# msalvaris/batchai_retinanet_horovod_coco

Measured on AMD Instinct MI355X. Metric: images/sec (whole node) RetinaNet-R50-FPN 800px at 1/2/4/8 MI355X, higher is better.
Workload: dtype bf16; 1 GPU; model=RetinaNet-R50-FPN, global_batch=16, per_gpu_batch=16, parallelism=dp1, clip_mode=global, allreduce_dtype=fp32, conv_backend=auto, hip_kernels=True, hip_graph=False, comm_engine=none, conv_table=/root/repo/tuning/conv_table.json, conv_raced=0, focal_fused_calls=101

## Files before the change

batchai_retinanet_horovod_coco_amd/models/retinanet.py:

```python
from __future__ import annotations

from typing import Dict, List, Optional, Sequence, Tuple

import os

import torch
import torch.nn as nn

from ..ops import anchors as anchor_ops
from ..ops import boxes as box_ops
from ..ops import conv as conv_ops
from ..ops import norm as norm_ops
from .layers import Conv2D, GroupNorm, prior_probability_bias
from .resnet import ResNet


class FPN(nn.Module):

    def __init__(self, c3: int, c4: int, c5: int, feature_size: int = 256):
        super().__init__()
        f = feature_size
        self.C5_reduced = Conv2D("C5_reduced", c5, f, 1, 1, "same")
        self.P5 = Conv2D("P5", f, f, 3, 1, "same")
        self.C4_reduced = Conv2D("C4_reduced", c4, f, 1, 1, "same")
        self.P4 = Conv2D("P4", f, f, 3, 1, "same")
        self.C3_reduced = Conv2D("C3_reduced", c3, f, 1, 1, "same")
        self.P3 = Conv2D("P3", f, f, 3, 1, "same")
        self.P6 = Conv2D("P6", c5, f, 3, 2, "same")
        self.P7 = Conv2D("P7", f, f, 3, 2, "same")

    def forward(self, C3, C4, C5, joins=None) -> List[torch.Tensor]:
        j = joins or {}
        P5r = self.C5_reduced(C5, join=j.get(3))
        P4m = conv_ops.upsample_add(P5r, self.C4_reduced(C4, join=j.get(2)))
        P3m = conv_ops.upsample_add(P4m, self.C3_reduced(C3, join=j.get(1)))
        P5 = self.P5(P5r)
        P4 = self.P4(P4m)
        P3 = self.P3(P3m)
        P6 = self.P6(C5, join=j.get(3))
        P7 = self.P7(torch.relu(P6))
        return [P3, P4, P5, P6, P7]

    def convs(self) -> List[Conv2D]:
        return [self.C5_reduced, self.P5, self.C4_reduced, self.P4, self.C3_reduced, self.P3, self.P6, self.P7]


HEAD_NORMS = (None, "gn")


def check_head_norm(head_norm, head_norm_groups: int, width: int = 256):
    if head_norm == "none":
        head_norm = None
    if head_norm not in HEAD_NORMS:
        raise ValueError("head_norm must be None or 'gn', got {!r}".format(head_norm))
    if head_norm == "gn" and (int(head_norm_groups) < 1 or width % int(head_norm_groups)):
        raise ValueError("head_norm_groups must divide the tower width {}, got {}".format(width, head_norm_groups))
    return head_norm


class Submodel(nn.Module):

    def __init__(self, name: str, prefix: str, cin: int, width: int, out_channels: int, final_bias: float,
                 head_norm: Optional[str] = None, head_norm_groups: int = 32):
        super().__init__()
        self.keras_name = name
        self.head_norm = check_head_norm(head_norm, head_norm_groups, width)
        self.tower = nn.ModuleList(
            [Conv2D(f"{prefix}_{i}", cin if i == 0 else width, width, 3, 1, "same", True, True, "normal001")
             for i in range(4)])
        self.final = Conv2D(prefix, width, out_channels, 3, 1, "same", True, False, "normal001", bias_value=final_bias)
        self.norms = None
        if self.head_norm == "gn":
            self.norms = nn.ModuleList([GroupNorm(f"{prefix}_{i}_gn", width, int(head_norm_groups)) for i in range(4)])
        if os.environ.get("MXR_HEAD_MAIN_WGRAD", "0") == "1":
            for c in self.convs():
                c.weight.mxr_main_wgrad = True

    def forward(self, feats: List[torch.Tensor]) -> List[torch.Tensor]:
        x = feats
        for i, c in enumerate(self.tower):
            w, b = c.effective(x[0].dtype)
            if self.norms is None:
                x = conv_ops.pyramid_conv(x, w, b, relu=True)
            else:
                n = self.norms[i]
                x = [norm_ops.group_norm_relu_nhwc(t, n.gamma, n.beta, n.groups, n.eps)
                     for t in conv_ops.pyramid_conv(x, w, b, relu=False)]
        w, b = self.final.effective(x[0].dtype)
        return conv_ops.pyramid_conv(x, w, b, relu=False)

    def forward_packed(self, x: torch.Tensor, shapes, pad_sink=None, join=None, chain=None) -> torch.Tensor:
        from ..ops import native_conv
        from ..ops import fp8
        if self.norms is not None:
            if fp8.enabled():
                raise RuntimeError("head_norm='gn' does not go with fp8: the tower layers hand fp8 copies of their "
                                   "ReLU outputs to each other")
            for i, (c, n) in enumerate(zip(self.tower, self.norms)):
                x = native_conv.pyramid_conv_layer(x, shapes, c, False, mask_input_grad=False, grad_premasked=False,
                                                   join=join if i == 0 else None, out_f8=False)
                x = norm_ops.group_norm_relu(x, shapes, n.gamma, n.beta, n.groups, n.eps)
            return native_conv.pyramid_conv_layer(x, shapes, self.final, False, mask_input_grad=False,
                                                  pad_sink=pad_sink)
        for i, c in enumerate(self.tower):
            nxt = self.tower[i + 1] if i + 1 < len(self.tower) else self.final
            x = native_conv.pyramid_conv_layer(x, shapes, c, True, mask_input_grad=i > 0, grad_premasked=True,
                                               join=join if i == 0 else None,
                                               out_f8=fp8.eligible(nxt.cin, nxt.cout),
                                               act=None if chain is None else (chain, len(self.tower) - i))
        return native_conv.pyramid_conv_layer(x, shapes, self.final, False, mask_input_grad=True,
                                              pad_sink=pad_sink, act=None if chain is None else (chain, 0))

    def convs(self) -> List[Conv2D]:
        return list(self.tower) + [self.final]


class RetinaNet(nn.Module):

    def __init__(self, num_classes: int, backbone: str = "resnet50", num_anchors: int = 9,
                 feature_size: int = 256, prior_probability: float = 0.01, head_norm: Optional[str] = None,
                 head_norm_groups: int = 32, regression_bins: int = 0, regression_range: float = 8.0):
        super().__init__()
        self.head_norm = check_head_norm(head_norm, head_norm_groups)
        self.head_norm_groups = int(head_norm_groups)
        self.regression_bins, self.regression_range = box_ops.check_regression_bins(regression_bins, regression_range)
        self.num_classes = num_classes
        self.num_anchors = num_anchors
        self.backbone_name = backbone
        if "resnet" in backbone:
            self.backbone = ResNet(backbone)
        else:
            from .extra_backbones import make_backbone
            self.backbone = make_backbone(backbone)
        c3, c4, c5 = self.backbone.out_channels[1:]
        self.fpn = FPN(c3, c4, c5, feature_size)
        self.regression_submodel = Submodel("regression_submodel", "pyramid_regression", feature_size, 256,
                                            num_anchors * 4 * max(1, self.regression_bins), 0.0, self.head_norm,
                                            self.head_norm_groups)
        self.classification_submodel = Submodel("classification_submodel", "pyramid_classification", feature_size,
                                                256, num_anchors * num_classes,
                                                prior_probability_bias(prior_probability), self.head_norm,
                                                self.head_norm_groups)

    def features(self, images: torch.Tensor) -> List[torch.Tensor]:
        joins = self._grad_joins(images)
        if joins is None:
            C3, C4, C5 = self.backbone(images)
            return self.fpn(C3, C4, C5)
        C3, C4, C5 = self.backbone(images, joins=joins)
        return self.fpn(C3, C4, C5, joins=joins if self.backbone.joins_active else None)

    def _grad_joins(self, images: torch.Tensor):
        if not (torch.is_grad_enabled() and isinstance(self.backbone, ResNet) and images.is_cuda
                and os.environ.get("MXR_GRAD_JOIN", "1") == "1" and conv_ops.get_conv_backend() != "torch"):
            return None
        from ..ops import native, native_conv
        if not native.available():
            return None
        dt = torch.bfloat16
        fpn = [self.fpn.C3_reduced, self.fpn.C4_reduced, self.fpn.C5_reduced, self.fpn.P6]
        if images.dtype != dt or not all(native_conv.hip_conv_ok(c.cin, c.cout, dt) for c in fpn):
            return None
        return {1: native_conv.GradJoin(2), 2: native_conv.GradJoin(2), 3: native_conv.GradJoin(2)}

    def forward(self, images: torch.Tensor) -> Dict[str, torch.Tensor]:
        feats = self.features(images)
        B = images.shape[0]
        if conv_ops.use_packed_heads(feats[0]):
            from ..ops import native
            packed, shapes = native.pyramid_pack(feats)
            from ..ops import native_conv
            join = native_conv.GradJoin(2) if (torch.is_grad_enabled() and
                                               os.environ.get("MXR_GRAD_JOIN", "1") == "1") else None
            self.reg_pad_sink = {} if torch.is_grad_enabled() else None
            from ..ops import fp8, row_activity
            chain = None
            if (torch.is_grad_enabled() and row_activity.enabled() and packed.dtype == torch.bfloat16
                    and self.head_norm is None and not fp8.enabled()):
                chain = row_activity.GradChain(len(self.regression_submodel.tower))
            reg = self.regression_submodel.forward_packed(packed, shapes, self.reg_pad_sink, join=join, chain=chain)
            self.cls_pad_sink = {} if torch.is_grad_enabled() else None
            req = getattr(self, "focal_request", None)
            if self.cls_pad_sink is not None and req is not None:
                self.cls_pad_sink["focal"] = req
            cls = self.classification_submodel.forward_packed(packed, shapes, self.cls_pad_sink, join=join)
            cls = cls.reshape(B, -1, self.num_classes)
            if self.regression_bins:
                return self._with_integral(reg.reshape(B, -1, 4 * self.regression_bins), cls)
            return {"regression": reg.reshape(B, -1, 4), "classification": cls}
        self.cls_pad_sink = self.reg_pad_sink = None
        reg = self.regression_submodel(feats)
        cls = self.classification_submodel(feats)
        classification = torch.cat([c.reshape(B, -1, self.num_classes) for c in cls], dim=1)
        if self.regression_bins:
            return self._with_integral(torch.cat([r.reshape(B, -1, 4 * self.regression_bins) for r in reg], dim=1),
                                       classification)
        regression = torch.cat([r.reshape(B, -1, 4) for r in reg], dim=1)
        return {"regression": regression, "classification": classification}

    def _with_integral(self, logits: torch.Tensor, classification: torch.Tensor) -> Dict[str, torch.Tensor]:
        K, R = self.regression_bins, self.regression_range
        state = getattr(self, "integral_request", None)
        if state is not None and logits.is_cuda:
            from ..ops import native
            try:
                regression = native.box_integral_fwd(logits.detach(), K, R, state=state)
                return {"regression": regression, "regression_logits": logits, "classification": classification}
            except native.NotServed:
                pass
        return {"regression": box_ops.box_integral(logits, K, R), "regression_logits": logits,
                "classification": classification}

    def convs(self) -> List[Conv2D]:
        return (self.backbone.convs() + self.fpn.convs() + self.regression_submodel.convs()
                + self.classification_submodel.convs())

    def pyramid_shapes(self, image_hw: Sequence[int]) -> List[Tuple[int, int]]:
        c = self.backbone.feature_shapes(image_hw)
        C3, C4, C5 = c[1], c[2], c[3]
        p6 = self.fpn.P6.out_hw(C5)
        p7 = self.fpn.P7.out_hw(p6)
        return [tuple(C3), tuple(C4), tuple(C5), tuple(p6), tuple(p7)]

    def backbone_parameters(self):
        return list(self.backbone.parameters())

    def norms(self) -> List[GroupNorm]:
        return [n for sub in (self.regression_submodel, self.classification_submodel) for n in (sub.norms or [])]

    def freeze_backbone(self) -> None:
        for p in self.backbone.parameters():
            p.requires_grad_(False)


class RetinaNetBBox(nn.Module):

    def __init__(self, model: RetinaNet, nms: bool = True, class_specific_filter: bool = True,
                 nms_threshold: float = 0.5, score_threshold: float = 0.05, max_detections: int = 300):
        super().__init__()
        self.model = model
        self.nms = nms
        self.class_specific_filter = class_specific_filter
        self.nms_threshold = nms_threshold
        self.score_threshold = score_threshold
        self.max_detections = max_detections
        self._anchors = anchor_ops.AnchorCache()

    @torch.no_grad()
    def forward(self, images: torch.Tensor):
        out = self.model(images)
        H, W = images.shape[1], images.shape[2]
        anchors = self._anchors.get((H, W), images.device, shapes_callback=anchor_ops.make_shapes_callback(self.model))
        from ..ops import native
        if (self.nms and self.class_specific_filter and images.is_cuda and native.available()
                and self.max_detections <= 512):
            return native.filter_detections_batched(anchors, out["regression"], out["classification"], H, W,
                                                    self.score_threshold, self.nms_threshold, self.max_detections)
        boxes = box_ops.bbox_transform_inv(anchors[None], out["regression"].float())
        boxes = box_ops.clip_boxes(boxes, H, W)
        cls = torch.sigmoid(out["classification"].float())
        res_b, res_s, res_l = [], [], []
        for i in range(images.shape[0]):
            b, s, l = box_ops.filter_detections(boxes[i], cls[i], self.nms, self.class_specific_filter,
                                                self.nms_threshold, self.score_threshold, self.max_detections)
            res_b.append(b)
            res_s.append(s)
            res_l.append(l)
        return torch.stack(res_b), torch.stack(res_s), torch.stack(res_l)


def retinanet_bbox(model: RetinaNet, **kwargs) -> RetinaNetBBox:
    return RetinaNetBBox(model, **kwargs)
```

batchai_retinanet_horovod_coco_amd/ops/conv_launch.py:

```python
from __future__ import annotations

import ctypes
import functools
import os
from typing import Callable, NamedTuple, Optional, Sequence, Tuple

import torch
import torch.nn.functional as F

from . import halo as _hx
from . import native as _n
from . import row_activity as _ra
from .native import ConvGeom, _chk, _p, _s, lib, zero_page, c_int, c_ll, c_vp
from .side_stream import SIDE


_SIGS = {
    "mxr_conv_wgrad": [c_vp, c_vp, c_int, c_vp, c_int, c_vp, c_vp, c_int, c_vp, ctypes.POINTER(ConvGeom), c_int, c_vp],
    "mxr_bias_grad": [c_vp, c_ll, c_int, c_int, c_int, c_vp, c_vp, c_vp, c_int, c_vp],
    "mxr_bias_res_act": [c_vp, c_vp, c_vp, c_ll, c_int, c_int, c_vp],
    "mxr_relu_bwd": [c_vp, c_vp, c_vp, c_ll, c_vp],
}

_BOUND = [False]
# ... 68 lines not shown
    @classmethod
    def of(cls, t: torch.Tensor) -> "BitMask":
        bm = cls(t)
        sh = torch.arange(8, device=t.device, dtype=torch.int32)
        bm.bits.copy_(((t.reshape(-1, 8) > 0).to(torch.int32) << sh).sum(1).to(torch.uint8))
        return bm

    def dense(self) -> torch.Tensor:
        sh = torch.arange(8, device=self.bits.device, dtype=torch.uint8)
        return ((self.bits[:, None] >> sh) & 1).bool().reshape(self.shape)

MASK_BITS = os.environ.get("MXR_MASK_BITS", "1") == "1"

FWD_VARIANTS = (0, 1, 2, 3, 4, 5, 6, 7, 8, 9, 10, 11, 12, 13, 14, 15, 16)
_IGEMM_VARIANTS = tuple(v for v in FWD_VARIANTS if v < 3)

def launch_hip(x, w, bias, res, y, g: ConvGeom, relu: bool, accumulate: bool = False, variant: int = 0,
               mask: Optional[torch.Tensor] = None) -> None:
    zp = _p(zero_page(x.device))
    if variant >= 3:
        return _chk(lib().mxr_conv_fwd_pipe(_p(x), _p(w), _p(bias), _p(res), _p(mask), _p(y), zp, ctypes.byref(g),
                                            int(relu), int(accumulate), variant - 3, _s()), "conv_fwd_pipe")
    _chk(lib().mxr_conv_fwd(_p(x), _p(w), _p(bias), _p(res), _p(mask), _p(y), zp, ctypes.byref(g), int(relu),
                            int(accumulate), variant, _s()), "conv_fwd")

HALO_VARIANTS = (0, 1, 2, 3, 4, 5, 6, 7, 8, 9, 10, 11, 12, 13, 14, 15)

HX32_VARIANTS = (0, 1, 2, 3, 4, 5, 6, 7, 8, 9, 10, 11, 12, 13, 14, 15)
HX32_NARROW = (8, 9)


NARROW_TILES = True


_HX32_WIDE = tuple(v for v in HX32_VARIANTS if v not in HX32_NARROW)

def hx32_variants(g: ConvGeom):
    return HX32_VARIANTS if g.cout <= 64 and NARROW_TILES else _HX32_WIDE

C1X1_BN = (64, 128, 256)

P8_VARIANTS = (0, 1, 2, 3, 4, 5, 6, 7, 8, 10)

P8_TUNED = (5, 6, 8)

def p8_covers(g: ConvGeom) -> bool:
    K = g.kh * g.kw * g.cin
    return (g.cin % 64 == 0 and g.cout % 8 == 0 and g.ostride == 1 and 1 <= g.nlev <= 5 and g.kh * g.kw <= 16
            and (int(g.M) + 1) * max(g.cin, g.cout) < 2 ** 31 and g.cout * K < 2 ** 31)

def big_tile_variants(g: ConvGeom):
    return ["p8_%d" % v for v in P8_TUNED] if p8_covers(g) else []

def launch_p8(x, w, bias, res, y, g: ConvGeom, relu: bool, accumulate: bool = False, variant: int = 0,
              mask: Optional[torch.Tensor] = None) -> None:
    if not p8_covers(g):
        raise RuntimeError("conv_p8: geometry not covered")
    K = g.kh * g.kw * g.cin
    if not (x.is_contiguous() and w.is_contiguous() and y.is_contiguous() and x.shape[-1] == g.cin
            and int(w.numel()) == g.cout * K and int(y.numel()) == int(g.M) * g.cout
            and (bias is None or bias.data_ptr() % 16 == 0)):
        raise RuntimeError("conv_p8: operand shapes do not match the geometry")
    _chk(lib().mxr_conv_p8(_p(x), _p(w), _p(bias), _p(res), _p(mask), _p(y), _p(zero_page(x.device)),
                           ctypes.byref(g), int(relu), int(accumulate), int(variant), _s()), "conv_p8")

SK_VARIANTS = (11, 12)


def splitk_splits(g: ConvGeom, v: int) -> int:
    if g.ostride != 1 or g.cin % 32 or g.cout % 8:
        return 0
    bco = 128 if v == 11 else 64
    tiles = -(-int(g.M) // 128) * -(-g.cout // bco)
    nks = g.kh * g.kw * g.cin // 32
    if tiles >= 256 or nks < 16:
        return 0
    s = min(64, max(2, round(512 / tiles)), nks // 8)
    return s if s >= 2 else 0


def launch_splitk(x, w, bias, res, y, g: ConvGeom, relu: bool, accumulate: bool = False, variant: int = 11,
                  mask: Optional[torch.Tensor] = None) -> None:
    ns = splitk_splits(g, variant)
    if ns < 2:
        raise RuntimeError("conv_fwd_pipe_sk: geometry not covered")
    part = torch.empty(ns * int(g.M) * g.cout, dtype=torch.float32, device=y.device)
    _chk(lib().mxr_conv_fwd_pipe_sk(_p(x), _p(w), _p(bias), _p(res), _p(mask), _p(y), _p(zero_page(x.device)),
                                    ctypes.byref(g), int(relu), int(accumulate), int(variant), ns, _p(part), _s()),
         "conv_fwd_pipe_sk")


def c1x1_variants(g: ConvGeom):
    if not (g.kh == 1 and g.kw == 1 and g.nlev == 1 and g.ostride == 1 and g.pt == 0 and g.pl == 0
            and g.stride in (1, 2) and g.cin in (64, 128, 256) and g.cout % 8 == 0):
        return []
    if g.stride == 1 and (g.H[0] != g.Ho[0] or g.W[0] != g.Wo[0]):
        return []
    eff = lambda bn: 64 if bn == 65 else bn
    return ["c1x1_%d" % bn for bn in C1X1_BN + (65,) if eff(bn) * g.cin <= 32768 and eff(bn) <= max(64, g.cout)]

def launch_c1x1(x, w, bias, res, y, g: ConvGeom, relu: bool, accumulate: bool = False, bn: int = 128,
                mask: Optional[torch.Tensor] = None) -> None:
    if "c1x1_%d" % bn not in c1x1_variants(g):
        raise RuntimeError("conv1x1_stream: geometry not covered")
    nimg = int(g.M) // (g.Ho[0] * g.Wo[0])
    if not (x.is_contiguous() and w.is_contiguous() and y.is_contiguous() and x.shape[-1] == g.cin
            and int(x.numel()) == nimg * g.H[0] * g.W[0] * g.cin and int(y.numel()) == int(g.M) * g.cout
            and int(w.numel()) == g.cout * g.cin and (bias is None or bias.data_ptr() % 16 == 0)):
        raise RuntimeError("conv1x1_stream: operand shapes do not match the geometry")
    _chk(lib().mxr_conv1x1_stream(_p(x), _p(w), _p(bias), _p(res), _p(mask), _p(y), int(g.M), g.cout, g.cin,
                                  g.H[0], g.W[0], g.Ho[0], g.Wo[0], g.stride, int(relu), int(accumulate), bn, 0,
                                  _s()), "conv1x1_stream")

def c1p_covers(g: ConvGeom) -> bool:
    return (g.kh == 1 and g.kw == 1 and g.nlev == 1 and g.ostride == 1 and g.pt == 0 and g.pl == 0
            and g.stride == 1 and g.H[0] == g.Ho[0] and g.W[0] == g.Wo[0] and g.cin % 32 == 0 and g.cin >= 96
            and g.cout % 8 == 0 and g.cout >= 64 and int(g.M) < 2 ** 31)

def launch_c1p(x, w, bias, res, y, g: ConvGeom, relu: bool, accumulate: bool = False,
               mask: Optional[torch.Tensor] = None) -> None:
    if not c1p_covers(g):
        raise RuntimeError("conv1x1_pers: geometry not covered")
    if not (x.is_contiguous() and w.is_contiguous() and y.is_contiguous() and x.shape[-1] == g.cin
            and int(x.numel()) == int(g.M) * g.cin and int(y.numel()) == int(g.M) * g.cout
            and int(w.numel()) == g.cout * g.cin and (bias is None or bias.data_ptr() % 16 == 0)
            and (res is None or (res.is_contiguous() and int(res.numel()) == int(g.M) * g.cout))):
        raise RuntimeError("conv1x1_pers: operand shapes do not match the geometry")
    _chk(lib().mxr_conv1x1_pers(_p(x), _p(w), _p(bias), _p(res), _p(mask), _p(y), _p(zero_page(x.device)),
                                _p(_n.trash_page(x.device)), int(g.M), g.cout, g.cin, int(relu), int(accumulate),
                                _s()), "conv1x1_pers")

def launch_halo(x, w, bias, res, y, g: ConvGeom, relu: bool, accumulate: bool = False, variant: int = 0,
                mask: Optional[torch.Tensor] = None) -> None:
    if not _hx.covers(g):
        raise RuntimeError("conv3x3_halo: geometry not covered")
    tiles, nt = _hx.device_tiles(_hx.geom_batch(g), _hx.geom_shapes(g), x.device)
    _chk(lib().mxr_conv3x3_halo(_p(x), _p(w), _p(bias), _p(res), _p(mask), _p(y), _p(zero_page(x.device)),
                                ctypes.byref(g), _p(tiles), nt, int(relu), int(accumulate), int(variant), _s()),
         "conv3x3_halo")

def launch_hx32(x, w, bias, res, y, g: ConvGeom, relu: bool, accumulate: bool = False, variant: int = 0,
                mask: Optional[torch.Tensor] = None, active=None) -> None:
    if not hx32_covers(g):
        raise RuntimeError("conv3x3_hx32: geometry not covered")
    if not (x.is_contiguous() and w.is_contiguous() and y.is_contiguous() and x.shape[-1] == g.cin
            and int(w.numel()) == g.cout * 9 * g.cin and int(y.numel()) == int(g.M) * g.cout
            and int(x.numel()) == int(g.M) * g.cin and (bias is None or bias.data_ptr() % 16 == 0)):
        raise RuntimeError("conv3x3_hx32: operand shapes do not match the geometry")
    if (g.cin // 32) % 2:
        variant = {2: 0, 3: 1, 13: 10, 14: 12}.get(variant, variant)
    tiles, nt = _hx.device_tiles(_hx.geom_batch(g), _hx.geom_shapes(g), x.device)
    wp = hx32_packed(w, g.cout, g.cin)
    act = active if active is not None else _ra.current()
    if act is not None and act.M == int(g.M) and act.ntiles == nt and bias is None and res is None and not relu:
        _ra.LAUNCHES["dgrad"] += 1
        return _chk(lib().mxr_conv3x3_hx32_act(_p(x), _p(wp), None, None, _p(mask), _p(y), _p(zero_page(x.device)),
                                               ctypes.byref(g), _p(tiles), nt, 0, int(accumulate), int(variant),
                                               _p(act.order), _p(act.count), _s()), "conv3x3_hx32_act")
    _chk(lib().mxr_conv3x3_hx32(_p(x), _p(wp), _p(bias), _p(res), _p(mask), _p(y), _p(zero_page(x.device)),
                                ctypes.byref(g), _p(tiles), nt, int(relu), int(accumulate), int(variant), _s()),
         "conv3x3_hx32")

class FocalRequest:

    def __init__(self, alpha: float = 0.25, gamma: float = 2.0):
        self.alpha, self.gamma = alpha, gamma
        self._buf = _n.ShapeSlots()
        self._qbuf = _n.ShapeSlots()
        self.set(None, None, None, 0)

    def set(self, state, label, npos, A: int) -> None:
        self.state, self.label, self.npos, self.A = state, label, npos, int(A)
        self.loss = None

    def dpad(self, n: int, p: int, ld: int, device) -> torch.Tensor:
        return self._buf.get((n, p, ld, str(device)),
                             lambda: torch.zeros((n, p, ld), dtype=torch.bfloat16, device=device))

    def dpad_q(self, n: int, p: int, ld: int, device) -> torch.Tensor:
        return self._qbuf.get((n, p, ld, str(device)),
                              lambda: torch.zeros((n, p, ld), dtype=torch.uint8, device=device))


FOCAL_FUSED = True
FOCAL_PREFER_MS = 0.15
FOCAL_LAUNCHES = [0]


FOCAL_VARIANTS = (0, 10)


def launch_hx32_focal(x, w, bias, g: ConvGeom, req: "FocalRequest", ld: int, variant: int = 0) -> torch.Tensor:
    from .losses import LOGIT_HI, LOGIT_LO
    N = int(g.M) // g.out_img
    C = g.cout // req.A
    if not (hx32_covers(g) and x.is_contiguous() and w.is_contiguous() and int(x.numel()) == int(g.M) * g.cin
            and int(w.numel()) == g.cout * 9 * g.cin and bias is not None and bias.data_ptr() % 16 == 0
            and C == 80 and req.gamma == 2.0 and ld % 8 == 0 and ld >= g.cout
            and int(req.state.numel()) == int(g.M) * req.A and int(req.label.numel()) == int(g.M) * req.A):
        raise RuntimeError("conv3x3_hx32_focal: operands do not match the geometry")
    tiles, nt = _hx.device_tiles(_hx.geom_batch(g), _hx.geom_shapes(g), x.device)
    wp = hx32_packed(w, g.cout, g.cin)
    nparts = -(-g.cout // 256) * nt
    parts = torch.empty(nparts, dtype=torch.float32, device=x.device)
    out = torch.empty(1, dtype=torch.float32, device=x.device)
    dpad = req.dpad(N, g.out_img, ld, x.device)
    if variant not in FOCAL_VARIANTS:
        raise RuntimeError("conv3x3_hx32_focal: no focal form of variant %r" % (variant,))
    _chk(lib().mxr_conv3x3_hx32_focal_v(_p(x), _p(wp), _p(bias), _p(zero_page(x.device)), ctypes.byref(g), _p(tiles),
                                        nt, _p(req.state.contiguous()), _p(req.label.contiguous()), _p(req.npos),
                                        _p(dpad), int(ld), req.A, C, float(req.alpha), float(req.gamma), LOGIT_LO,
                                        LOGIT_HI, _p(parts), nparts, _p(out), int(variant), _s()),
         "conv3x3_hx32_focal")
    req.loss = out.reshape(())
    FOCAL_LAUNCHES[0] += 1
    return dpad

def hx32_packed(w: torch.Tensor, cout: int, cin: int) -> torch.Tensor:
    cw = _n.compute_weights()
    if cw is not None:
        wp = cw.hx32_packed(w)
        if wp is not None:
            return wp
    wp = torch.empty(cout * 9 * cin, dtype=w.dtype, device=w.device)
    _chk(lib().mxr_hx32_pack_weights(_p(w), _p(wp), cout, cin, _s()), "hx32_pack")
    return wp

def hx32_covers(g: ConvGeom) -> bool:
    return _hx.covers(g) and g.cout * 9 * g.cin * 2 < 2 ** 31


class Family(NamedTuple):
    prefix: str
    names: Callable
    launch: Callable
    bits: object

def _numbered(prefix: str, fn):
    n = len(prefix)
    return lambda *a: fn(*a[:8], int(a[8][n:]), a[9])

@functools.lru_cache(maxsize=None)
def _named(prefix: str, variants) -> Tuple[str, ...]:
    return tuple("%s%d" % (prefix, v) for v in variants)

FAMILIES = (
    Family("hip", lambda g: _named("hip", FWD_VARIANTS if g.cout % 8 == 0 else _IGEMM_VARIANTS),
           _numbered("hip", launch_hip), lambda name: name[3:].isdigit() and int(name[3:]) >= 3),
    Family("halo", lambda g: _named("halo", HALO_VARIANTS) if _hx.covers(g) else (), _numbered("halo", launch_halo), True),
    Family("hx32_", lambda g: _named("hx32_", hx32_variants(g)) if hx32_covers(g) else (),
           _numbered("hx32_", launch_hx32), True),
    Family("c1x1_", c1x1_variants, _numbered("c1x1_", launch_c1x1), True),
    Family("c1p", lambda g: ("c1p",) if c1p_covers(g) else (), lambda *a: launch_c1p(*a[:8], a[9]), True),
    Family("p8_", big_tile_variants, _numbered("p8_", launch_p8), False),
    Family("sk", lambda g: _named("sk", tuple(v for v in SK_VARIANTS if splitk_splits(g, v))),
           _numbered("sk", launch_splitk), True),
)
_FAMILY = {f.prefix: f for f in FAMILIES}

FWD_ORDER = ("hip", "halo", "hx32_", "c1x1_", "c1p", "p8_", "sk")
DGRAD_ORDER = ("hip", "c1x1_", "c1p", "p8_", "halo", "hx32_")
DGRAD_S2_ORDER = ("hip",)
DGRAD_SKIP = ("c1x1_65",)

def family_of(name: str) -> Optional[Family]:
    return _FAMILY.get(name.rstrip("0123456789"))

def offered(g: ConvGeom, order=FWD_ORDER, skip=()):
    return [n for p in order for n in _FAMILY[p].names(g) if n not in skip]

def bits_capable(name: str) -> bool:
    bits = getattr(family_of(name), "bits", False)
    return bits(name) if callable(bits) else bits

def _bits_filter(cands, mask):
    if not isinstance(mask, BitMask):
        return cands
    return {k: v for k, v in cands.items() if bits_capable(k)}

def launch_fwd(x, w, bias, res, y, g: ConvGeom, relu: bool, accumulate: bool = False,
               variant=None, mask: Optional[torch.Tensor] = None) -> None:
    v = _variant(g.cout) if variant is None else variant
    if not isinstance(v, str):
        return launch_hip(x, w, bias, res, y, g, relu, accumulate, v, mask)
    fam = family_of(v)
    if fam is None:
        raise RuntimeError("launch_fwd: %r names no kernel family" % (v,))
    fam.launch(x, w, bias, res, y, g, relu, accumulate, v, mask)

def relu_bwd_(dy: torch.Tensor, y: torch.Tensor) -> torch.Tensor:
    assert dy.is_contiguous() and y.is_contiguous() and dy.shape == y.shape
    _chk(_bind().mxr_relu_bwd(_p(dy), _p(y), _p(dy), dy.numel(), _s()), "relu_bwd_")
    return dy

def relu_bwd(dy: torch.Tensor, y: torch.Tensor) -> torch.Tensor:
    dx = torch.empty_like(dy)
    _chk(_bind().mxr_relu_bwd(_p(dy), _p(y), _p(dx), dy.numel(), _s()), "relu_bwd")
    return dx

def bias_res_act_(y: torch.Tensor, bias: Optional[torch.Tensor], res: Optional[torch.Tensor], relu: bool):
    if bias is None and res is None and not relu:
        return y
    _chk(_bind().mxr_bias_res_act(_p(y), _p(bias), _p(res), y.numel(), y.shape[-1], int(relu), _s()), "epilogue")
    return y

def miopen_fwd(x, w, bias, res, stride, pads, relu):
    pt, pb, pl, pr = pads
# ... 206 lines not shown
```

batchai_retinanet_horovod_coco_amd/ops/halo.py:

```python
from __future__ import annotations

from typing import Dict, List, Sequence, Tuple

import numpy as np

HX_BOX = 4
HX_HMAX = 448
HX_PB = 256
COLMAX = 84
NFIELD = 10
TILE_INTS = 4 + HX_BOX * NFIELD


def _split(n: int, parts: int) -> List[Tuple[int, int]]:
    out, start = [], 0
    for i in range(parts):
        ln = n // parts + (1 if i < n % parts else 0)
        out.append((start, ln))
        start += ln
    return out


def level_boxes(H: int, W: int) -> List[Tuple[int, int, int, int]]:
    cols = _split(W, -(-W // COLMAX))
    cmax = max(c for _, c in cols)
    R = max(1, min(H, HX_PB // cmax))
    while R > 1 and (R + 2) * (cmax + 2) > HX_HMAX:
        R -= 1
    boxes = []
    for y0 in range(0, H, R):
        r = min(R, H - y0)
        for x0, c in cols:
            boxes.append((y0, r, x0, c))
    return boxes


def build_tiles(N: int, shapes: Sequence[Tuple[int, int]], open_tiles: int = 4) -> np.ndarray:
    img = sum(h * w for h, w in shapes)
    offs, o = [], 0
    for h, w in shapes:
        offs.append(o)
        o += h * w
    per_level = [level_boxes(h, w) for h, w in shapes]
    tiles: List[dict] = []
    open_idx: List[int] = []
    for b in range(N):
        for lv, (H, W) in enumerate(shapes):
            base = b * img + offs[lv]
            for (y0, R, x0, C) in per_level[lv]:
                ns, nh = R * C, (R + 2) * (C + 2)
                di = None
                for ti in open_idx:
                    t = tiles[ti]
                    if len(t["boxes"]) < HX_BOX and t["nslot"] + ns <= HX_PB and t["nhalo"] + nh <= HX_HMAX:
                        di = ti
                        break
                if di is None:
                    tiles.append({"boxes": [], "nslot": 0, "nhalo": 0})
                    di = len(tiles) - 1
                    open_idx.append(di)
                    if len(open_idx) > open_tiles:
                        open_idx.pop(0)
                t = tiles[di]
                t["boxes"].append((t["nslot"], t["nhalo"], base, base, H, W, y0, x0, R, C))
                t["nslot"] += ns
                t["nhalo"] += nh
                if (t["nslot"] > HX_PB - 16 or len(t["boxes"]) == HX_BOX) and di in open_idx:
                    open_idx.remove(di)
    out = np.zeros((len(tiles), TILE_INTS), dtype=np.int32)
    for i, t in enumerate(tiles):
        out[i, 0:3] = (len(t["boxes"]), t["nslot"], t["nhalo"])
        for k, bx in enumerate(t["boxes"]):
            out[i, 4 + k * NFIELD:4 + (k + 1) * NFIELD] = bx
    return out


def _boxes(row) -> List[Tuple[int, ...]]:
    return [tuple(int(v) for v in row[4 + k * NFIELD:4 + (k + 1) * NFIELD]) for k in range(int(row[0]))]


def check_tiles(tab: np.ndarray, N: int, shapes: Sequence[Tuple[int, int]]) -> None:
    total = N * sum(h * w for h, w in shapes)
    seen = np.zeros(total, dtype=np.int32)
    for row in tab:
        nbox, nslot, nhalo = int(row[0]), int(row[1]), int(row[2])
        assert 1 <= nbox <= HX_BOX and nslot <= HX_PB and nhalo <= HX_HMAX, row[:4]
        s = h = 0
        for (sbeg, hoff, ib, ob, H, W, y0, x0, R, C) in _boxes(row):
            assert sbeg == s and hoff == h and ib == ob
            assert 0 <= y0 and y0 + R <= H and 0 <= x0 and x0 + C <= W
            for r in range(R):
                seen[ob + (y0 + r) * W + x0:ob + (y0 + r) * W + x0 + C] += 1
            s += R * C
            h += (R + 2) * (C + 2)
        assert s == nslot and h == nhalo
    assert (seen == 1).all(), "pixels covered {} .. {} times".format(seen.min(), seen.max())


def waste(tab: np.ndarray, N: int, shapes: Sequence[Tuple[int, int]]) -> float:
    return 1.0 - N * sum(h * w for h, w in shapes) / float(len(tab) * HX_PB)


def emulate(x: np.ndarray, w: np.ndarray, tab: np.ndarray) -> np.ndarray:
    P, cin = x.shape
    cout = w.shape[0]
    y = np.zeros((P, cout), dtype=np.float64)
    for row in tab:
        nslot, nhalo = int(row[1]), int(row[2])
        boxes = _boxes(row)
        halo = np.zeros((HX_HMAX, cin))
        for h in range(nhalo):
            k = max(i for i in range(len(boxes)) if h >= boxes[i][1])
            sbeg, hoff, ib, ob, H, W, y0, x0, R, C = boxes[k]
            hr, hc = divmod(h - hoff, C + 2)
            yy, xx = y0 - 1 + hr, x0 - 1 + hc
            if 0 <= yy < H and 0 <= xx < W:
                halo[h] = x[ib + yy * W + xx]
        for p in range(nslot):
            k = max(i for i in range(len(boxes)) if p >= boxes[i][0])
            sbeg, hoff, ib, ob, H, W, y0, x0, R, C = boxes[k]
            r, c = divmod(p - sbeg, C)
            pw = C + 2
            hb = hoff + r * pw + c
            acc = np.zeros(cout)
            for ky in range(3):
                for kx in range(3):
                    acc += w[:, ky, kx, :] @ halo[hb + ky * pw + kx]
            y[ob + (y0 + r) * W + x0 + c] = acc
    return y



def pack_row_bits(rows: np.ndarray) -> np.ndarray:
    P = int(rows.shape[0])
    pad = np.zeros((P + 63) // 64 * 64, dtype=np.uint64)
    pad[:P] = rows.astype(np.uint64)
    return (pad.reshape(-1, 64) << np.arange(64, dtype=np.uint64)).sum(axis=1, dtype=np.uint64)


def unpack_row_bits(words: np.ndarray, P: int) -> np.ndarray:
    w = np.asarray(words).view(np.uint64).reshape(-1, 1)
    return ((w >> np.arange(64, dtype=np.uint64)) & np.uint64(1)).astype(bool).reshape(-1)[:P]


def dilate_rows(rows: np.ndarray, N: int, shapes: Sequence[Tuple[int, int]]) -> np.ndarray:
    out = np.zeros_like(rows, dtype=bool)
    img = sum(h * w for h, w in shapes)
    for b in range(N):
        off = b * img
        for h, w in shapes:
            a = rows[off:off + h * w].reshape(h, w).astype(bool)
            p = np.zeros((h + 2, w + 2), dtype=bool)
            p[1:-1, 1:-1] = a
            d = np.zeros((h, w), dtype=bool)
            for dy in range(3):
                for dx in range(3):
                    d |= p[dy:dy + h, dx:dx + w]
            out[off:off + h * w] = d.reshape(-1)
            off += h * w
    return out


def active_tiles(tab: np.ndarray, rows: np.ndarray) -> np.ndarray:
    act = np.zeros(len(tab), dtype=bool)
    for i, row in enumerate(tab):
        for (sbeg, hoff, ib, ob, H, W, y0, x0, R, C) in _boxes(row):
            ya, yb = max(0, y0 - 1), min(H - 1, y0 + R)
            xa, xb = max(0, x0 - 1), min(W - 1, x0 + C)
            lv = rows[ob:ob + H * W].reshape(H, W)
            if lv[ya:yb + 1, xa:xb + 1].any():
                act[i] = True
                break
    return act


def tile_rows(tab: np.ndarray, which: np.ndarray, P: int) -> np.ndarray:
    out = np.zeros(P, dtype=bool)
    for row in tab[np.asarray(which, dtype=bool)]:
        for (sbeg, hoff, ib, ob, H, W, y0, x0, R, C) in _boxes(row):
            for r in range(R):
                out[ob + (y0 + r) * W + x0:ob + (y0 + r) * W + x0 + C] = True
    return out


_CACHE: Dict[tuple, object] = {}


def device_tiles(N: int, shapes: Sequence[Tuple[int, int]], device):
    import torch
    key = (str(device), int(N), tuple((int(h), int(w)) for h, w in shapes), COLMAX)
    hit = _CACHE.get(key)
    if hit is None:
        tab = build_tiles(N, key[2])
        hit = (torch.from_numpy(tab).to(device), int(tab.shape[0]))
        _CACHE[key] = hit
    return hit


def geom_shapes(g) -> List[Tuple[int, int]]:
    return [(int(g.H[l]), int(g.W[l])) for l in range(int(g.nlev))]


def geom_batch(g) -> int:
    return int(g.M // max(1, g.out_img))


def covers(g) -> bool:
    if not (g.kh == 3 and g.kw == 3 and g.stride == 1 and g.pt == 1 and g.pl == 1 and g.ostride == 1):
        return False
    if g.cin % 32 or g.cout % 8:
        return False
    if any(g.H[l] != g.Ho[l] or g.W[l] != g.Wo[l] for l in range(g.nlev)):
        return False
    if g.in_img != g.out_img:
        return False
    return (g.M + 1) * max(g.cin, g.cout) < 2 ** 31
```

batchai_retinanet_horovod_coco_amd/ops/native.py:

```python
from __future__ import annotations

import ctypes
import os
from typing import List, Optional, Sequence, Tuple

import torch
import torch.nn.functional as F

_HERE = os.path.dirname(os.path.abspath(__file__))
_PKG = os.path.dirname(_HERE)
LIB_PATH = os.environ.get("MXR_KERNEL_LIB") or os.path.join(_PKG, "_lib", "libmxr_kernels.so")

_LIB: Optional[ctypes.CDLL] = None
_DISABLED = [os.environ.get("MXR_DISABLE_KERNELS", "0") == "1"]
_LOAD_ERR: List[str] = []

c_int, c_ll, c_float, c_vp = ctypes.c_int, ctypes.c_longlong, ctypes.c_float, ctypes.c_void_p

MAXLEV = 5


class ConvGeom(ctypes.Structure):
    _fields_ = [("nlev", c_int), ("H", c_int * MAXLEV), ("W", c_int * MAXLEV), ("Ho", c_int * MAXLEV),
                ("Wo", c_int * MAXLEV), ("in_off", c_int * MAXLEV), ("mstart", c_int * (MAXLEV + 1)),
                ("in_img", c_int), ("out_img", c_int), ("stride", c_int), ("pt", c_int), ("pl", c_int),
                ("kh", c_int), ("kw", c_int), ("cin", c_int), ("cout", c_int), ("M", c_ll),
                ("ostride", c_int), ("oH", c_int), ("oW", c_int), ("ooy", c_int), ("oox", c_int)]


_SIGS = {
    "mxr_focal_fwd_bwd": [c_vp, c_vp, c_vp, c_vp, c_vp, c_vp, c_vp, c_ll, c_int, c_float, c_float, c_float, c_float,
                          c_int, c_int, c_int, c_vp],
    "mxr_smooth_l1_fwd_bwd": [c_vp, c_vp, c_vp, c_vp, c_vp, c_vp, c_vp, c_ll, c_float, c_int, c_int, c_int, c_vp],
    "mxr_iou_loss_fwd_bwd": [c_vp, c_vp, c_vp, c_vp, c_vp, c_vp, c_vp, c_vp, c_ll, c_int, c_int, c_float, c_int, c_int,
                             c_int, c_vp],
    "mxr_quality_loss_fwd_bwd": [c_vp, c_vp, c_vp, c_vp, c_vp, c_vp, c_vp, c_vp, c_vp, c_vp, c_ll, c_int, c_int, c_int,
                                 c_int, c_int, c_int, c_vp],
    "mxr_box_integral_fwd": [c_vp, c_vp, c_vp, c_ll, c_int, c_float, c_int, c_vp],
    "mxr_box_dist_fwd_bwd": [c_vp, c_vp, c_vp, c_vp, c_vp, c_vp, c_vp, c_vp, c_ll, c_int, c_float, c_float, c_int, c_int,
                             c_int, c_vp],
    "mxr_loss_grid": [],
    "mxr_gn_chunk_rows": [],
    "mxr_gn_relu_fwd": [c_vp] * 7 + [c_ll, c_int, c_ll, c_int, c_int, c_float, c_int, ctypes.POINTER(c_int), c_int, c_vp],
    "mxr_gn_relu_bwd": [c_vp] * 10 + [c_ll, c_int, c_ll, c_int, c_int, c_int, ctypes.POINTER(c_int), c_int, c_vp],
    "mxr_anchor_targets": [c_vp, c_vp, c_int, c_vp, c_int, c_int, c_vp, c_vp, c_vp, c_vp, c_vp, c_vp, c_float, c_float,
                           c_float, c_vp],
    "mxr_atss_targets": [c_vp, c_vp, c_int, ctypes.POINTER(c_int), c_int, c_vp, c_int, c_int, c_vp, c_vp, c_int, c_vp,
                         c_vp, c_vp, c_vp, c_vp, c_vp, c_vp, c_float, c_vp],
    "mxr_chunk_struct_sizes": [c_vp],
    "mxr_adam_step": [c_vp, c_vp, c_vp, c_vp, c_vp, c_vp, c_vp, c_int, c_vp, c_vp, c_vp, c_vp, c_float, c_float,
                      c_float, c_vp],
    "mxr_sgd_step": [c_vp, c_vp, c_vp, c_vp, c_vp, c_vp, c_int, c_vp, c_vp, c_vp, c_vp, c_vp, c_int, c_vp],
    "mxr_refresh_copy": [c_vp, c_vp, c_vp, c_vp, c_int, c_vp, c_vp],
    "mxr_adam_step_ema": [c_vp, c_vp, c_vp, c_vp, c_vp, c_vp, c_vp, c_vp, c_int, c_vp, c_vp, c_vp, c_vp, c_float,
                          c_float, c_float, c_float, c_ll, c_vp],
    "mxr_sgd_step_ema": [c_vp, c_vp, c_vp, c_vp, c_vp, c_vp, c_vp, c_int, c_vp, c_vp, c_vp, c_vp, c_vp, c_int,
                         c_float, c_ll, c_vp],
    "mxr_swap_refresh": [c_vp, c_vp, c_vp, c_vp, c_vp, c_int, c_vp, c_vp],
    "mxr_grad_norm_clip": [c_vp, c_ll, c_vp, c_float, c_float, c_float, c_vp, c_vp],
    "mxr_scale_inplace": [c_vp, c_ll, c_vp, c_vp],
    "mxr_norm_grid": [],
    "mxr_maxpool_fwd": [c_vp, c_vp, c_vp] + [c_int] * 11 + [c_int, c_int, c_vp],
    "mxr_wgrad3x3_c64": [c_vp] * 5 + [c_int] * 4 + [c_vp],
    "mxr_wgrad_halo": [c_vp, c_vp, c_int, c_vp, c_int, c_int, c_int, c_int, c_vp, c_vp, c_vp, c_vp, c_vp, c_int, c_int, c_int,
                       c_vp, c_vp, c_vp, c_int, c_vp],
    "mxr_flip_batch": [c_vp, c_vp, c_vp, c_vp, c_int, c_vp],
    "mxr_conv1x1_stream": [c_vp] * 6 + [c_int] * 12 + [c_vp],
    "mxr_conv1x1_pers_dual": [c_vp] * 9 + [c_ll, c_int, c_int, c_int, c_int, c_int, c_int, c_int, c_int, c_vp],
    "mxr_conv1x1_pers": [c_vp] * 8 + [c_ll, c_int, c_int, c_int, c_int, c_vp],
    "mxr_conv_wgrad_p8_f8": [c_vp, c_vp, c_int, c_vp, c_vp, c_vp, c_int, c_vp, c_vp, c_int, c_vp,
                             ctypes.POINTER(ConvGeom), c_int, c_vp],
    "mxr_hx8_quant_pack_batch": [c_vp, c_int, c_int, c_vp],
    "mxr_conv_wgrad_p8_f8_bias": [c_vp, c_vp, c_int, c_vp, c_vp, c_vp, c_int, c_vp, c_vp, c_int, c_vp,
                                  ctypes.POINTER(ConvGeom), c_int, c_vp, c_int, c_vp],
    "mxr_stem_fwd": [c_vp, c_vp, c_vp, c_vp] + [c_int] * 8 + [c_vp],
    "mxr_stem_pool_fwd": [c_vp, c_vp, c_vp, c_vp, c_vp] + [c_int] * 11 + [c_vp],
    "mxr_stem_pack": [c_vp, c_vp, c_vp, c_vp],
    "mxr_stem_wgrad": [c_vp, c_vp, c_vp, c_vp, c_vp] + [c_int] * 8 + [c_vp] + [c_int] * 4 + [c_vp],
    "mxr_maxpool_bwd": [c_vp, c_vp, c_vp] + [c_int] * 10 + [c_int, c_vp],
    "mxr_upsample_add_fwd": [c_vp, c_vp, c_vp, c_vp, c_vp] + [c_int] * 6 + [c_int, c_vp],
    "mxr_upsample_bwd": [c_vp, c_vp, c_vp, c_vp] + [c_int] * 6 + [c_int, c_vp],
    "mxr_decode_clip": [c_vp, c_vp, c_int, c_vp, c_int, c_int, c_float, c_float, c_float, c_vp],
    "mxr_nms": [c_vp, c_int, c_float, c_int, c_vp, c_vp, c_vp, c_vp],
    "mxr_filter_select": [c_vp, c_int, c_int, c_int, c_int, c_float, c_vp, c_vp, c_int, c_vp],
    "mxr_filter_nms": [c_vp, c_vp, c_int, c_int, c_int, c_int, c_vp, c_vp, c_int, c_int, c_int, c_float, c_float,
                       c_float, c_float, c_int, c_vp, c_vp, c_vp, c_vp, c_vp],
    "mxr_conv_geom_size": [],
    "mxr_s2_stack_flip": [c_vp, c_vp, c_int, c_int, c_vp, c_vp],
    "mxr_conv_fwd": [c_vp, c_vp, c_vp, c_vp, c_vp, c_vp, c_vp, ctypes.POINTER(ConvGeom), c_int, c_int, c_int, c_vp],
    "mxr_conv_fwd_pipe": [c_vp, c_vp, c_vp, c_vp, c_vp, c_vp, c_vp, ctypes.POINTER(ConvGeom), c_int, c_int, c_int,
                          c_vp],
    "mxr_conv_fwd_pipe_dual": [c_vp, c_vp, c_int, c_int, c_int, c_int, c_int, c_vp, c_vp, c_vp, c_vp, c_vp, c_vp,
                               ctypes.POINTER(ConvGeom), c_int, c_int, c_vp],
    "mxr_conv_dgrad_pipe_dd": [c_vp, c_vp, c_vp, c_vp, c_vp, c_vp, c_int, c_int, c_int, c_int, c_int, c_int, c_vp,
                               ctypes.POINTER(ConvGeom), c_int, c_vp],
    "mxr_conv_fwd_pipe_sk": [c_vp, c_vp, c_vp, c_vp, c_vp, c_vp, c_vp, ctypes.POINTER(ConvGeom), c_int, c_int, c_int,
                             c_int, c_vp, c_vp],
    "mxr_conv_p8": [c_vp, c_vp, c_vp, c_vp, c_vp, c_vp, c_vp, ctypes.POINTER(ConvGeom), c_int, c_int, c_int, c_vp],
    "mxr_conv3x3_halo": [c_vp, c_vp, c_vp, c_vp, c_vp, c_vp, c_vp, ctypes.POINTER(ConvGeom), c_vp, c_int, c_int, c_int,
                         c_int, c_vp],
    "mxr_hx32_pack_weights": [c_vp, c_vp, c_int, c_int, c_vp],
    "mxr_hx32_pack_batch": [c_vp, c_int, c_vp, c_ll, c_vp],
    "mxr_conv3x3_hx32": [c_vp, c_vp, c_vp, c_vp, c_vp, c_vp, c_vp, ctypes.POINTER(ConvGeom), c_vp, c_int, c_int, c_int,
                         c_int, c_vp],
    "mxr_conv_wgrad_p8": [c_vp, c_vp, c_int, c_vp, c_int, c_vp, c_vp, c_int, c_vp, ctypes.POINTER(ConvGeom), c_int,
                          c_vp],
    "mxr_conv_wgrad_p8_dual": [c_vp, c_vp, c_int, c_vp, c_int, c_vp, c_int, c_vp, c_vp, c_vp, c_vp, c_int, c_vp,
                               ctypes.POINTER(ConvGeom), c_int, c_vp],
    "mxr_conv_wgrad_p8_bias": [c_vp, c_vp, c_int, c_vp, c_int, c_vp, c_vp, c_int, c_vp, ctypes.POINTER(ConvGeom),
                               c_int, c_vp, c_int, c_vp],
    "mxr_conv3x3_hx32_act": [c_vp, c_vp, c_vp, c_vp, c_vp, c_vp, c_vp, ctypes.POINTER(ConvGeom), c_vp, c_int, c_int,
                             c_int, c_int, c_vp, c_vp, c_vp],
    "mxr_conv_wgrad_p8_bias_act": [c_vp, c_vp, c_int, c_vp, c_int, c_vp, c_vp, c_int, c_vp, ctypes.POINTER(ConvGeom),
                                   c_int, c_vp, c_int, c_vp, c_vp],
    "mxr_rows_nonzero": [c_vp, c_ll, c_int, c_vp, c_vp],
    "mxr_rows_dilate": [c_vp, c_vp, c_int, c_ll, ctypes.POINTER(ConvGeom), c_vp],
    "mxr_halo_active_tiles": [c_vp, c_int, c_vp, c_ll, c_int, c_vp, c_vp, c_vp],
    "mxr_conv_wgrad_pipe": [c_vp, c_vp, c_int, c_vp, c_int, c_vp, c_vp, c_int, c_vp, ctypes.POINTER(ConvGeom), c_int,
                            c_vp],
    "mxr_conv_wgrad_pipe_direct": [c_vp, c_vp, c_int, c_vp, c_vp, c_int, c_vp, ctypes.POINTER(ConvGeom), c_int, c_vp],
    "mxr_flip_transpose": [c_vp, c_vp, c_int, c_int, c_int, c_int, c_vp],
    "mxr_image_warp_normalize": [c_vp, c_int, c_int, c_vp, c_int, c_int, c_vp, c_int, c_int, c_int, c_float, c_float,
                                 c_float, c_float, c_float, c_vp],
    "mxr_image_resize_into": [c_vp, c_int, c_int, c_vp, c_int, c_int, c_ll, c_int, c_vp],
    "mxr_image_batch_resize_normalize": [c_vp, c_ll, c_vp, c_int, c_vp, c_int, c_int, c_int, c_int, c_float, c_float,
                                         c_float, c_float, c_vp],
    "mxr_image_batch_warp_resize_normalize": [c_vp, c_ll, c_vp, c_vp, c_int, c_vp, c_int, c_int, c_int, c_int, c_int,
                                              c_int, c_float, c_float, c_float, c_float, c_float, c_vp],
    "mxr_detections_finish": [c_vp, c_vp, c_vp, c_vp, c_int, c_int, c_float, c_vp, c_vp, c_vp],
    "mxr_fp8_amax": [c_vp, c_ll, c_vp, c_vp],
    "mxr_fp8_quant": [c_vp, c_ll, c_vp, c_vp, c_vp, c_vp],
    "mxr_fp8_quant_rows": [c_vp, c_int, c_int, c_vp, c_vp, c_vp],
    "mxr_conv_fwd_f8": [c_vp, c_vp, c_vp, c_vp, c_vp, c_vp, c_vp, c_vp, ctypes.POINTER(ConvGeom), c_int, c_vp, c_vp,
                        c_vp, c_int, c_float, c_int, c_vp],
    "mxr_conv_p8_f8": [c_vp, c_vp, c_vp, c_vp, c_vp, c_vp, c_vp, c_vp, c_vp, ctypes.POINTER(ConvGeom), c_int, c_int,
                       c_vp, c_vp, c_vp, c_int, c_float, c_int, c_vp],
    "mxr_bf8_quant": [c_vp, c_ll, c_vp, c_vp, c_vp, c_vp],
    "mxr_quant_delayed": [c_vp, c_ll, c_vp, c_vp, c_int, c_float, c_vp, c_int, c_vp],
    "mxr_hx8_pack_weights": [c_vp, c_vp, c_int, c_int, c_vp],
    "mxr_hx8_quant_pack": [c_vp, c_int, c_int, c_vp, c_vp, c_vp],
    "mxr_conv3x3_hx32_f8": [c_vp, c_vp, c_vp, c_vp, c_vp, c_vp, c_vp, c_vp, c_vp, ctypes.POINTER(ConvGeom), c_vp, c_int,
                            c_int, c_int, c_vp, c_vp, c_vp, c_int, c_float, c_int, c_vp],
    "mxr_conv3x3_hx32_focal": [c_vp, c_vp, c_vp, c_vp, ctypes.POINTER(ConvGeom), c_vp, c_int, c_vp, c_vp, c_vp, c_vp,
                               c_int, c_int, c_int, c_float, c_float, c_float, c_float, c_vp, c_int, c_vp, c_vp],
    "mxr_conv3x3_hx32_focal_v": [c_vp, c_vp, c_vp, c_vp, ctypes.POINTER(ConvGeom), c_vp, c_int, c_vp, c_vp, c_vp, c_vp,
                                 c_int, c_int, c_int, c_float, c_float, c_float, c_float, c_vp, c_int, c_vp, c_int,
                                 c_vp],
    "mxr_conv3x3_hx32_f8_focal": [c_vp, c_vp, c_vp, c_vp, c_vp, c_vp, ctypes.POINTER(ConvGeom), c_vp, c_int, c_vp, c_vp,
                                  c_vp, c_vp, c_int, c_int, c_int, c_float, c_float, c_float, c_float, c_vp, c_int, c_vp,
                                  c_vp],
    "mxr_conv3x3_hx32_f8_focal_q": [c_vp, c_vp, c_vp, c_vp, c_vp, c_vp, ctypes.POINTER(ConvGeom), c_vp, c_int, c_vp,
                                    c_vp, c_vp, c_vp, c_int, c_int, c_int, c_float, c_float, c_float, c_float, c_vp,
                                    c_int, c_vp, c_vp, c_vp, c_vp, c_int, c_float, c_vp],
    "mxr_s2_shuffle": [c_vp, c_vp, c_vp, c_int, c_int, c_int, c_int, c_int, c_int, c_int, c_vp],
    "mxr_s2_stack": [c_vp, c_vp, c_int, c_int, c_vp, c_vp],
    "mxr_pyr_pack": [c_vp, c_vp, c_vp, c_int, c_int, c_int, c_int, c_vp],
    "mxr_pyr_pack_f8": [c_vp, c_vp, c_vp, c_int, c_int, c_int, c_vp, c_vp, c_vp, c_int, c_float, c_vp],
}
_OPTIONAL = {"mxr_conv_wgrad", "mxr_bias_grad", "mxr_relu_bwd"}


def load(required: bool = False, check_device: bool = True) -> bool:
    global _LIB
    if _LIB is not None:
        return True
    if not os.path.exists(LIB_PATH):
        msg = "HIP kernel library not built: {} (run python -m batchai_retinanet_horovod_coco_amd.build)".format(LIB_PATH)
        _LOAD_ERR.append(msg)
        if required:
            raise RuntimeError(msg)
        return False
    try:
        lib = ctypes.CDLL(LIB_PATH)
        for name, args in _SIGS.items():
            fn = getattr(lib, name)
            fn.argtypes = args
            fn.restype = c_int
        if lib.mxr_conv_geom_size() != ctypes.sizeof(ConvGeom):
            raise RuntimeError("ConvGeom layout mismatch ({} vs {})".format(lib.mxr_conv_geom_size(),
                                                                         ctypes.sizeof(ConvGeom)))
    except Exception as e:
        _LOAD_ERR.append(str(e))
        if required:
            raise
        return False
    _LIB = lib
    return True


def disable() -> None:
    _DISABLED[0] = True


def enable() -> None:
    _DISABLED[0] = False


def available() -> bool:
    if _DISABLED[0] or not torch.cuda.is_available():
        return False
    return load(required=os.environ.get("MXR_REQUIRE_KERNELS", "1") == "1")


def conv_supported() -> bool:
    return available() and os.environ.get("MXR_HIP_CONV", "1") == "1"


def loaded_libraries() -> List[str]:
    return [LIB_PATH] if _LIB is not None else []


def lib() -> ctypes.CDLL:
    if _LIB is None:
        load(required=True)
    return _LIB


_RAW_STREAM = getattr(torch._C, "_cuda_getCurrentRawStream", None)
_CUR_DEV = getattr(torch._C, "_cuda_getDevice", None)


def _s() -> int:
    if _RAW_STREAM is not None:
        return _RAW_STREAM(_CUR_DEV())
    return torch.cuda.current_stream().cuda_stream


def _p(t: Optional[torch.Tensor]):
    return None if t is None else t.data_ptr()


_SYNC_DEBUG = os.environ.get("MXR_SYNC_DEBUG", "0") == "1"


def _chk(rc: int, name: str) -> None:
    if rc != 0:
        raise RuntimeError("{} failed with code {}".format(name, rc))
    if _SYNC_DEBUG:
        try:
            torch.cuda.synchronize()
        except RuntimeError as e:
            raise RuntimeError("{} faulted: {}".format(name, e)) from e


def _dt(t: torch.Tensor) -> int:
    if t.dtype == torch.bfloat16:
        return 1
    if t.dtype == torch.float32:
        return 0
    raise TypeError("unsupported dtype {}".format(t.dtype))


_ZERO = {}


def zero_page(device) -> torch.Tensor:
    key = str(device)
    z = _ZERO.get(key)
    if z is None:
        z = torch.zeros(256, dtype=torch.uint8, device=device)
        _ZERO[key] = z
    return z


_TRASH = {}


def trash_page(device) -> torch.Tensor:
    key = str(device)
    t = _TRASH.get(key)
# ... 1119 lines not shown
```

batchai_retinanet_horovod_coco_amd/ops/native_conv.py:

```python
from __future__ import annotations

import ctypes
import os
from typing import Optional, Sequence, Tuple

import torch
import torch.nn.functional as F

from . import native as _n
from .native import ConvGeom, _chk, _p, _s, lib, zero_page, c_int, c_ll, c_vp
from .side_stream import SIDE
from . import row_activity as _ra
from .conv_launch import (
    MASK_BITS, BitMask, bits_capable, proj_fusable, run_fwd_proj, run_fwd_into, C1X1_BN, FWD_VARIANTS, HALO_VARIANTS, HX32_VARIANTS, P8_TUNED, P8_VARIANTS, _BOUND, _SIGS, _bind,
    _effective, _miopen_pyramid_wgrad, _miopen_wgrad, _only, _out_hw, _variant, bias_res_act_,
    big_tile_variants, c1x1_variants, family_of, flip, fwd_candidates, geom_pyramid, geom_single, hip_conv_ok,
    hx32_covers, hx32_packed, launch_c1x1, launch_fwd, launch_halo, launch_hx32, launch_p8, miopen_fwd,
    p8_covers, relu_bwd, relu_bwd_, run_fwd, torch_conv_backward,)
from .conv_dgrad import (
    proj_dgrad_fusable, run_dgrad_proj, _dgrad_cands, _dgrad_s2_subpixel, _pick_taps, _s2_phase_taps, _s2_stack_taps,
    _s2_stacked_weights, _s2_stacked_weights_hip, conv_dgrad, run_dgrad,)
from .conv_wgrad import (
    proj_wgrad_fusable, run_wgrad_proj, _WGRAD_P8, _WGRAD_PIPE_OCC, _WGRAD_PIPE_TILE, _WGRAD_TILE, _WGRAD_VS, _WH_TILES, _deliver_wgrad,
    _only_wgrad, _sink, _splits, _splits_pipe, _wgrad_sink_cands, _wh_box, bias_grad, conv_wgrad,
# ... 134 lines not shown
                    h = run_fwd_proj(h, x, w2c, w1, b2c + b1, st1, emit=emit)
                else:
                    shortcut = run_fwd(x, w1, b1, None, st1, specs[nconv][1], False)
                    h = run_fwd(h, w2c, b2c, shortcut, st, pd, True, emit=emit)
            else:
                h = run_fwd(h, ws[i][0], ws[i][1], shortcut if last else None, st, pd, True, emit=emit if last else None)
            hs.append(h)
        if emit is not None:
            h._mxr_bits = emit
        ctx.specs = specs
        ctx.nconv = nconv
        ctx.has_b1 = specs[nconv] is not None
        ctx.wparams = [params[3 * i] for i in range(nconv + 1)]
        present = [i for i in range(nconv + 1) if ws[i] is not None]
        ctx.save_for_backward(*(hs + [ws[i][0] for i in present] + [scales[i] for i in present]))
        return h

    @staticmethod
    def backward(ctx, dout):
        specs, nconv = ctx.specs, ctx.nconv
        saved = ctx.saved_tensors
        hs = saved[:nconv + 1]
        nw = nconv + (1 if ctx.has_b1 else 0)
        ws = list(saved[nconv + 1:nconv + 1 + nw])
        scs = list(saved[nconv + 1 + nw:])
        out = hs[-1]
        g = dout.to(out.dtype).contiguous()
        if not ctx.premasked:
            g = relu_bwd(g, out)
        elif g is dout and not ctx.has_b1 and ctx.needs_input_grad[0] and not _INPLACE_GRAD:
            g = g.clone()
        grads = [None] * (3 * (nconv + 1))
        need_x = ctx.needs_input_grad[0]
        dx = None
        jbuf, mask_in = None, ctx.mask_in
        if ctx.join is not None and need_x:
            jbuf, _ = ctx.join.claim()
            mask_in = True
        dh_last = None
        wfused = False
        if ctx.has_b1:
            st, pd = specs[nconv]
            if (ctx.needs_input_grad[4 + 3 * nconv] and ctx.needs_input_grad[4 + 3 * (nconv - 1)] and nconv >= 2
                    and specs[nconv - 1] == (1, (0, 0, 0, 0)) and pd == (0, 0, 0, 0)
                    and proj_wgrad_fusable(hs[nconv - 1], hs[0], g, ws[nconv - 1], ws[nconv], st)):
                wfused = run_wgrad_proj(hs[nconv - 1], hs[0], g, st, scs[nconv - 1], scs[nconv],
                                        ctx.wparams[nconv - 1], ctx.wparams[nconv])
            if ctx.needs_input_grad[4 + 3 * nconv] and not wfused:
                grads[3 * nconv] = run_wgrad(hs[0], g, ws[nconv], st, pd, scs[nconv], param=ctx.wparams[nconv])
            if need_x:
                if (nconv >= 2 and specs[nconv - 1] == (1, (0, 0, 0, 0)) and pd == (0, 0, 0, 0) and
                        proj_dgrad_fusable(g, ws[nconv - 1], ws[nconv], hs[nconv - 1], tuple(hs[0].shape), st)):
                    dh_last, dx = run_dgrad_proj(g, ws[nconv - 1], ws[nconv], hs[nconv - 1], tuple(hs[0].shape), st,
                                                 out=jbuf)
                else:
                    dx = run_dgrad(g, ws[nconv], hs[0], st, pd, out=jbuf)
        gi = g
        for i in range(nconv - 1, -1, -1):
            st, pd = specs[i]
            if ctx.needs_input_grad[4 + 3 * i] and not (wfused and i == nconv - 1):
                grads[3 * i] = run_wgrad(hs[i], gi, ws[i], st, pd, scs[i], param=ctx.wparams[i])
            if i > 0:
                if i == nconv - 1 and dh_last is not None:
                    gi = dh_last
                    continue
                gi = run_dgrad(gi, ws[i], hs[i], st, pd, mask=hs[i])
            elif need_x:
                mk = hs[0] if mask_in else None
                if mk is not None and ctx.bits_in is not None and ws[0].shape[1] == 1:
                    mk = ctx.bits_in
                if dx is None and jbuf is None and st == 1 and SIDE.usable(g):
                    dx = run_dgrad(gi, ws[0], hs[0], st, pd, res=g, mask=mk)
                else:
                    if dx is None:
                        if jbuf is not None:
                            dx = jbuf.add_(g)
                        else:
                            dx = g if gi is not g else g.clone()
                    dx = run_dgrad(gi, ws[0], hs[0], st, pd, out=dx, mask=mk)
        if ctx.join is not None and need_x:
            if jbuf is None:
                ctx.join.buf = dx
            else:
                if dx is not jbuf:
                    jbuf.copy_(dx)
                ctx.join.release()
                dx = None
        return (dx, None, None, None) + tuple(grads)

_BLOCK_CHUNK = int(os.environ.get("MXR_BLOCK_CHUNK", "0"))
_BLOCK_CHUNK_MIN_PX = int(os.environ.get("MXR_BLOCK_CHUNK_MIN_PX", "10000"))


def _block_chunk(x, specs) -> int:
    if (_BLOCK_CHUNK <= 0 or specs[-1] is not None or x.shape[0] < 2 * _BLOCK_CHUNK
            or x.shape[1] * x.shape[2] < _BLOCK_CHUNK_MIN_PX or any(st != 1 for st, _ in specs[:-1])):
        return 0
    return _BLOCK_CHUNK


def _bits_view(full: BitMask, i0: int, i1: int) -> BitMask:
    v = BitMask.__new__(BitMask)
    per = full.bits.numel() // full.shape[0]
    v.bits = full.bits[i0 * per:i1 * per]
    v.shape = (i1 - i0,) + tuple(full.shape[1:])
    v.device = full.device
    return v


def _chunked_chain(x, ws, specs, nconv, cout, bits_ok, chunk):
    N, H, W, _ = x.shape
    outs = [torch.empty((N, H, W, ws[i][0].shape[0]), dtype=x.dtype, device=x.device) for i in range(nconv)]
    emit = BitMask(shape=(N, H, W, cout), device=x.device) if bits_ok else None
    for i0 in range(0, N, chunk):
        i1 = min(N, i0 + chunk)
        xs = x[i0:i1]
        h = xs
        for i in range(nconv):
            st, pd = specs[i]
            last = i == nconv - 1
            em = _bits_view(emit, i0, i1) if (last and emit is not None) else None
            h = run_fwd_into(outs[i][i0:i1], h, ws[i][0], ws[i][1], xs if last else None, st, pd, True, emit=em)
    if emit is not None:
        outs[-1]._mxr_bits = emit
    return outs


def residual_block(x, convs, branch1, mask_input_grad: bool = False, grad_premasked: bool = False,
                   join: Optional[GradJoin] = None) -> torch.Tensor:
    specs, params = [], []
    hw = tuple(x.shape[1:3])
    for c in convs:
        specs.append((c.stride, tuple(c.pads(hw))))
        hw = c.out_hw(hw)
    specs.append(None if branch1 is None else (branch1.stride, tuple(branch1.pads(tuple(x.shape[1:3])))))
    for c in list(convs) + [branch1]:
        if c is None:
            params += [None, None, None]
            continue
        sc, sh = c.bn.scale_shift() if c.bn is not None else (None, None)
        params += [c.weight, sc, sh]
    return ResidualBlockFn.apply(x, tuple(specs), (bool(mask_input_grad), bool(grad_premasked)), join, *params)

def fused_block_ok(x, convs) -> bool:
    return (os.environ.get("MXR_FUSED_BLOCKS", "1") == "1" and x.is_cuda and x.dtype == torch.bfloat16
            and all(c is None or (hip_conv_ok(c.cin, c.cout, x.dtype) and c.bias is None) for c in convs))

HEAD_BITS = True

class PyramidConvFn(torch.autograd.Function):

    @staticmethod
    def forward(ctx, x, weight, bias, shapes, relu, mask_input_grad=False, grad_premasked=False, pad_sink=None,
                join=None, out_f8=False, act=None):
        from .conv_tuner import TUNER
        ctx.act = act
        x = x.contiguous()
        N, P, cin = x.shape
        cout = weight.shape[0]
        w, b = _effective(weight, None, bias, None)
        ctx.wdt = weight.dtype
        g = geom_pyramid(N, shapes, cin, cout)
        from . import fp8 as _f8
        ctx.f8x = None
        f8_only_in = getattr(x, "_mxr_f8only", False)
        ctx.bits_in = getattr(x, "_mxr_bits", None) if mask_input_grad else None
        if f8_only_in and not (_f8.enabled() and _f8.eligible(cin, cout) and _f8.WGRAD and ctx.bits_in is not None):
            raise RuntimeError("PyramidConvFn: the input is an fp8-only tower output; this layer would read its bf16 "
                               "values")
        if _f8.enabled() and _f8.eligible(cin, cout):
            from . import conv_launch as _cl
            req = pad_sink.get("focal") if pad_sink is not None else None
            if not (req is not None and req.state is not None and _cl.FOCAL_FUSED and req.A > 0):
                req = None
            y = _f8.pyramid_forward(x, w, b, g, relu, (N, P, cout), weight,
                                    TUNER.key("pfwd", N, tuple(shapes), cin, cout, int(relu)) + "|f8",
                                    f8_only=bool(out_f8) and _f8.WGRAD and _f8.F8_ONLY_TOWERS and MASK_BITS
                                    and relu and any(ctx.needs_input_grad), focal=req,
                                    focal_dq_ok=bool(weight.requires_grad and _f8.WGRAD
                                                     and (bias is None or _f8.bias_fusable(weight, bias))))
            if getattr(y, "_mxr_focal_dpad", None) is not None:
                pad_sink["dy"] = y._mxr_focal_dpad
            if weight.requires_grad and _f8.WGRAD:
                ctx.f8x = _f8.quantize_cached(x)
                if getattr(y, "_mxr_f8only", False):
                    y._mxr_grad_f8ok = bias is None or _f8.bias_fusable(weight, bias)
        elif _focal_fused(pad_sink, relu, b, g, TUNER.key("pfwd", N, tuple(shapes), cin, cout, int(relu))):
            from .conv_launch import launch_hx32_focal
            req = pad_sink["focal"]
            fv = 10 if TUNER.winner(TUNER.key("pfwd", N, tuple(shapes), cin, cout, int(relu))) == "hx32_10" else 0
            pad_sink["dy"] = launch_hx32_focal(x, w, b, g, req, (cout + 63) // 64 * 64, variant=fv)
            y = torch.empty((N, P, cout), dtype=x.dtype, device=x.device)
            y._mxr_unwritten = True
        else:
            emit = BitMask(shape=(N, P, cout), device=x.device) if (
                relu and MASK_BITS and HEAD_BITS and x.is_cuda and cout % 8 == 0 and any(ctx.needs_input_grad)) else None
            key = TUNER.key("pfwd", N, tuple(shapes), cin, cout, int(relu)) + ("|eb" if emit is not None else "")
            cands = fwd_candidates(x, w, b, None, g, 1, (1, 1, 1, 1), relu, (N, P, cout), allow_miopen=False,
                                   mask=emit)
            if cout % 8 and cout < 64:
                cands["pad64"] = lambda: _pad64_pfwd(x, w, b, shapes, relu)
            y = TUNER.run(key, cands)
            if emit is not None:
                y._mxr_bits = emit
        ctx.save_for_backward(x, w, y if relu else None)
        ctx.params = (weight, bias)
        ctx.cfg = (tuple(shapes), relu, bias is not None, bool(mask_input_grad), bool(grad_premasked))
        ctx.pad_sink = pad_sink
        ctx.join = join
        return y

    @staticmethod
    def backward(ctx, dy):
        from .conv_tuner import TUNER
        x, w, y = ctx.saved_tensors
        shapes, relu, has_bias, mask_in, premasked = ctx.cfg
        N, P, cin = x.shape
        cout = w.shape[0]
        padded = ctx.pad_sink.pop("dy", None) if ctx.pad_sink is not None else None
        if padded is not None:
            dy = padded
        else:
            dy = dy.to(x.dtype).contiguous()
        from . import fp8 as _f8
        dy_f8only = getattr(dy, "_mxr_f8only", False)
        if dy_f8only and not ((premasked or not relu) and ctx.f8x is not None and _f8.cache_get(dy) is not None
                              and (not has_bias or _f8.bias_fusable(ctx.params[0], ctx.params[1]))):
            raise RuntimeError("PyramidConvFn: the incoming gradient is an fp8-only data gradient; this layer would "
                               "read its bf16 values")
        if relu and not premasked:
            dy = relu_bwd(dy, y)
        dx = dw = db = None
        mk = None
        if mask_in:
            mk = ctx.bits_in if ctx.bits_in is not None else x
        ract = wact = None
        if ctx.act is not None and ctx.f8x is None:
            chain, depth_k = ctx.act
            if depth_k == 0:
                chain.start(dy, N, shapes)
            ract = chain.level(depth_k)
            wact = ract if depth_k > 0 else None
        f8_only_in = getattr(x, "_mxr_f8only", False)
        from . import fp8 as _f8
        f8dy = None
        if ctx.f8x is not None and ctx.needs_input_grad[1]:
            dq_src = dy
            if cout % 64 and dq_src.shape[-1] % 64:
                cp = (cout + 63) // 64 * 64
                dq_src = F.pad(dy, (0, cp - dy.shape[-1]))
            f8dy = _f8.quantize_bf8_cached(dq_src, key=("dyq", ctx.params[0]))
            if ctx.needs_input_grad[0] and cout % 64 and dq_src is not dy:
                dy = dq_src
        if ctx.needs_input_grad[0]:
            wd = flip(w)
            dyp = dy
            if cout % 64:
                cp = (cout + 63) // 64 * 64
                if dyp.shape[-1] != cp:
                    dyp = F.pad(dy, (0, cp - cout))
                wd = F.pad(wd, (0, cp - cout))
            wd = wd.contiguous()
            gd = geom_pyramid(N, shapes, dyp.shape[-1], cin)
            key = TUNER.key("pdgrad", N, tuple(shapes), cin, cout) + ("|mb" if isinstance(mk, BitMask) else "")
            buf = None
            if ctx.join is not None:
                buf, _ = ctx.join.claim()
            from . import fp8 as _f8
            if _f8.enabled() and _f8.dgrad_eligible(dyp.shape[-1], cin):
                f8o = f8_only_in and _f8.F8_ONLY_DGRAD and getattr(x, "_mxr_grad_f8ok", False)
                r = _f8.pyramid_dgrad(dyp, wd, gd, mk, (N, P, cin), ("pdgrad", ctx.params[0]),
                                      key + ("|a" if buf is not None else "") + "|f8", emit=mask_in, out=buf,
                                      f8_only=f8o)
                if buf is None:
                    dx = r
                    if ctx.join is not None:
                        ctx.join.buf = dx
                else:
                    ctx.join.release()
                    dx = None
            elif buf is None:
                with _ra.using(ract):
                    dx = TUNER.run(key, fwd_candidates(dyp, wd, None, None, gd, 1, (1, 1, 1, 1), False, (N, P, cin),
                                                       allow_miopen=False, mask=mk))
                if ctx.join is not None:
                    ctx.join.buf = dx
            else:
                cands = fwd_candidates(dyp, wd, None, None, gd, 1, (1, 1, 1, 1), False, (N, P, cin),
                                       allow_miopen=False, mask=mk, out=buf)
                if TUNER.needs_tuning(key + "|a", cands):
                    TUNER.run(key + "|a", fwd_candidates(dyp, wd, None, None, gd, 1, (1, 1, 1, 1), False,
                                                         (N, P, cin), allow_miopen=False, mask=mk, out=buf.clone()))
                with _ra.using(ract):
                    TUNER.run(key + "|a", cands)
                ctx.join.release()
                dx = None
        fused_bias = False
        if ctx.needs_input_grad[1]:
            gw = geom_pyramid(N, shapes, cin, cout)
            wkey = TUNER.key("pwgrad", N, tuple(shapes), cin, cout)
            if f8dy is not None and _f8.wgrad_eligible(gw, int(f8dy[0].shape[-1])):
                fb = has_bias and ctx.needs_input_grad[2] and _f8.bias_fusable(ctx.params[0], ctx.params[1])
                dw = _f8.deliver_pyramid_wgrad(ctx.f8x, f8dy, gw, ctx.params[0], reads=(x, dy),
                                               bias_param=ctx.params[1] if fb else None)
                if dw is not None:
                    dw = dw.to(ctx.wdt)
                if has_bias and ctx.needs_input_grad[2] and not fb:
                    db = deliver_bias_grad(ctx.params[1], dy, channels=cout)
                return dx, dw, db, None, None, None, None, None, None, None, None
            with _ra.using(wact):
                fused_bias = (has_bias and ctx.needs_input_grad[2]
                              and deliver_wgrad_bias_fused(wkey, x, dy, gw, ctx.params[0], ctx.params[1]))
        if f8_only_in and ctx.needs_input_grad[1]:
            raise RuntimeError("PyramidConvFn: a bf16 weight gradient over an fp8-only tower output")
        if ctx.needs_input_grad[1] and not fused_bias:
            cands = wgrad_candidates(x, dy, gw, None)
            dyl = dy if dy.shape[-1] == cout else dy[..., :cout]
            lib_fn = lambda: _miopen_pyramid_wgrad(x, w, dyl, shapes)
            cands["miopen"] = lib_fn
            sink_make = _wgrad_sink_cands(x, dy, gw, None, lib_fn)
            if cout % 8 and cout < 64:
                narrow = {"pad64": lambda: _pad64_pwgrad(x, dy, shapes, cout)}
                if SWAP_NARROW_WGRAD:
                    narrow["swap"] = lambda: _swap_pwgrad(x, dy, shapes, cout)
                cands.update(narrow)
                base_make = sink_make

                def sink_make(sink, only=None, base_make=base_make, narrow=narrow):
                    if only in narrow:
                        return {only: lambda: sink.add_(narrow[only]())}
                    c = base_make(sink, only)
                    if only is None:
                        c.update({n: (lambda fn=fn: sink.add_(fn())) for n, fn in narrow.items()})
                    return c
            with _ra.using(wact):
                dw = _deliver_wgrad(wkey, cands, sink_make, ctx.params[0], (x, dy))
            if dw is not None:
                dw = dw.to(ctx.wdt)
        if has_bias and ctx.needs_input_grad[2] and not fused_bias:
            db = deliver_bias_grad(ctx.params[1], dy, channels=cout)
        return dx, dw, db, None, None, None, None, None, None, None, None

def _focal_fused(pad_sink, relu, b, g: ConvGeom, key: str) -> bool:
    from . import conv_launch as _cl
    from .conv_tuner import TUNER
    req = pad_sink.get("focal") if pad_sink is not None else None
    return (req is not None and req.state is not None and _cl.FOCAL_FUSED and not relu and b is not None
            and req.A > 0 and g.cout == 80 * req.A and _cl.hx32_covers(g)
            and (TUNER.prefer(key, "hx32_10", _cl.FOCAL_PREFER_MS) or TUNER.prefer(key, "hx32_0", _cl.FOCAL_PREFER_MS)))

def _pad64_pfwd(x, w, b, shapes, relu):
    from .conv_tuner import TUNER
    N, P, cin = x.shape
    cout = w.shape[0]
    wp = F.pad(w, (0, 0, 0, 0, 0, 0, 0, 64 - cout)).contiguous()
    bp = None if b is None else F.pad(b, (0, 64 - cout)).contiguous()
    gp = geom_pyramid(N, shapes, cin, 64)
    yp = TUNER.run(TUNER.key("pfwd", N, tuple(shapes), cin, 64, int(relu), "pad"),
                   fwd_candidates(x, wp, bp, None, gp, 1, (1, 1, 1, 1), relu, (N, P, 64), allow_miopen=False))
    return yp[..., :cout].contiguous()

def _pad64_pwgrad(x, dy, shapes, cout):
    from .conv_tuner import TUNER
    N, P, cin = x.shape
    dyp = dy if dy.shape[-1] == 64 else F.pad(dy[..., :cout], (0, 64 - cout)).contiguous()
    gp = geom_pyramid(N, shapes, cin, 64)
    dw = TUNER.run(TUNER.key("pwgrad", N, tuple(shapes), cin, 64, "pad"), wgrad_candidates(x, dyp, gp, None))
    return dw[:cout]

SWAP_NARROW_WGRAD = True

def _swap_pwgrad(x, dy, shapes, cout):
    from .conv_tuner import TUNER
    N, P, cin = x.shape
    dyp = dy if dy.shape[-1] == 64 else F.pad(dy[..., :cout], (0, 64 - cout)).contiguous()
    gs = geom_pyramid(N, shapes, 64, cin)
    r = TUNER.run(TUNER.key("pwgrad", N, tuple(shapes), 64, cin, "swap"), wgrad_candidates(dyp, x, gs, None))
    return r[..., :cout].flip(1, 2).permute(3, 1, 2, 0)

def conv_layer(x, layer, residual=None, relu=None, join: Optional[GradJoin] = None) -> torch.Tensor:
    relu = layer.relu if relu is None else relu
    pads = layer.pads(x.shape[1:3])
    scale = shift = None
    if layer.bn is not None:
        scale, shift = layer.bn.scale_shift()
    if not hip_conv_ok(layer.cin, layer.cout, x.dtype):
        if join is not None:
            raise RuntimeError("GradJoin consumer %s is not on the HIP conv path" % layer.keras_name)
        from .conv import _conv_torch
        w, b = layer.effective(x.dtype)
        return _conv_torch(x, w, b, layer.stride, pads, relu, residual)
    return ConvLayerFn.apply(x, layer.weight, layer.bias, scale, shift, layer.stride, tuple(pads), bool(relu),
                             residual, join)

def _pyr_pack(packed: torch.Tensor, levels, shapes, unpack: bool) -> None:
    ptrs = (c_vp * 5)(*([t.data_ptr() for t in levels] + [None] * (5 - len(levels))))
    hw = (c_int * 5)(*([h * w for h, w in shapes] + [0] * (5 - len(shapes))))
    _chk(lib().mxr_pyr_pack(_p(packed), ptrs, hw, len(levels), packed.shape[0], packed.shape[-1], int(unpack), _s()),
         "pyr_pack")

class PyramidPackFn(torch.autograd.Function):

    @staticmethod
    def forward(ctx, *xs):
        N, C = xs[0].shape[0], xs[0].shape[-1]
        shapes = tuple((int(x.shape[1]), int(x.shape[2])) for x in xs)
        ctx.shapes = shapes
        packed = torch.empty((N, sum(h * w for h, w in shapes), C), dtype=xs[0].dtype, device=xs[0].device)
        from . import fp8 as _f8
        if _f8.enabled():
            st = _f8.amax_state("pyr_features", packed.device)
            yq = torch.empty(packed.shape, dtype=torch.uint8, device=packed.device) if st.ready else None
            inv = torch.empty(1, dtype=torch.float32, device=packed.device)
            levels = [x.contiguous() for x in xs]
            ptrs = (c_vp * 5)(*([t.data_ptr() for t in levels] + [None] * (5 - len(levels))))
            hw = (c_int * 5)(*([h * w for h, w in shapes] + [0] * (5 - len(shapes))))
            _chk(lib().mxr_pyr_pack_f8(_p(packed), ptrs, hw, len(levels), N, C, _p(yq), _p(st.amax3), _p(inv),
                                       int(st.phase), float(_f8.MARGIN), _s()), "pyr_pack_f8")
            if yq is not None:
                _f8.cache_put(packed, yq, inv)
            st.advance()
            return packed
        _pyr_pack(packed, [x.contiguous() for x in xs], shapes, False)
        return packed

    @staticmethod
    def backward(ctx, dp):
        dp = dp.contiguous()
        N, C = dp.shape[0], dp.shape[-1]
        outs = [torch.empty((N, h, w, C), dtype=dp.dtype, device=dp.device) for h, w in ctx.shapes]
        _pyr_pack(dp, outs, ctx.shapes, True)
        return tuple(outs)

def pyramid_pack(xs: Sequence[torch.Tensor]):
    N = xs[0].shape[0]
    C = xs[0].shape[-1]
    shapes = tuple((int(x.shape[1]), int(x.shape[2])) for x in xs)
    if (xs[0].is_cuda and xs[0].dtype == torch.bfloat16 and C % 8 == 0 and 1 <= len(xs) <= 5
            and all(x.dtype == xs[0].dtype and x.shape[0] == N and x.shape[-1] == C for x in xs)):
        return PyramidPackFn.apply(*xs), shapes
    packed = torch.cat([x.reshape(N, -1, C) for x in xs], dim=1)
    return packed, shapes

def pyramid_conv_layer(x, shapes, layer, relu, mask_input_grad=False, grad_premasked=False,
                       pad_sink=None, join=None, out_f8: bool = False, act=None) -> torch.Tensor:
    return PyramidConvFn.apply(x, layer.weight, layer.bias, tuple(shapes), bool(relu), bool(mask_input_grad),
                               bool(grad_premasked), pad_sink, join, bool(out_f8), act)

def pyramid_unpack(y, shapes):
    out, off = [], 0
    N = y.shape[0]
    for (h, wd) in shapes:
        out.append(y[:, off:off + h * wd].reshape(N, h, wd, -1))
        off += h * wd
    return out



class _RawConvFn(torch.autograd.Function):
    @staticmethod
    def forward(ctx, x, w, bias, stride, pads, relu, residual):
        ctx.wdt = w.dtype
        return ConvLayerFn.forward(ctx, x, w.float(), bias, None, None, stride, pads, relu, residual)

    @staticmethod
    def backward(ctx, dy):
        dx, dw, db, *_rest, dres = ConvLayerFn.backward(ctx, dy)
        return dx, (None if dw is None else dw.to(ctx.wdt)), db, None, None, None, dres

def conv2d(x, w, bias, stride, pads, relu, residual):
    if not hip_conv_ok(x.shape[-1], w.shape[0], x.dtype):
        from .conv import _conv_torch
        return _conv_torch(x, w, bias, stride, pads, relu, residual)
    return _RawConvFn.apply(x, w, bias, stride, tuple(pads), bool(relu), residual)

def pyramid_conv_packed(x, shapes, w, bias, relu):
    return PyramidConvFn.apply(x, w, bias, tuple(shapes), bool(relu))

def pyramid_conv(xs, w, bias, relu):
    packed, shapes = pyramid_pack(xs)
    return pyramid_unpack(pyramid_conv_packed(packed, shapes, w, bias, relu), shapes)
```

batchai_retinanet_horovod_coco_amd/ops/row_activity.py:

```python
from __future__ import annotations

import ctypes
import os
from typing import Dict, Optional, Sequence, Tuple

import torch

from . import halo as _hx
from .native import ConvGeom, _chk, _p, _s, lib

MAX_DEPTH = 8
LAUNCHES = {"dgrad": 0, "wgrad": 0}


def enabled() -> bool:
    return os.environ.get("MXR_SPARSE_REG_GRAD", "1") == "1"


class Activity:
    __slots__ = ("words", "order", "count", "M", "ntiles")

    def __init__(self, words, order, count, M, ntiles):
        self.words, self.order, self.count, self.M, self.ntiles = words, order, count, int(M), int(ntiles)


_CUR = [None]


class using:
    __slots__ = ("act", "prev")

    def __init__(self, act: Optional[Activity]):
        self.act, self.prev = act, None

    def __enter__(self):
        self.prev, _CUR[0] = _CUR[0], self.act
        return self.act

    def __exit__(self, *exc):
        _CUR[0] = self.prev
        return False


def current() -> Optional[Activity]:
    return _CUR[0]


def rows_nonzero(dy: torch.Tensor, out: Optional[torch.Tensor] = None) -> torch.Tensor:
    ld = int(dy.shape[-1])
    rows = dy.numel() // ld
    if not (dy.is_cuda and dy.dtype == torch.bfloat16 and dy.is_contiguous() and ld % 8 == 0):
        raise RuntimeError("rows_nonzero: a contiguous bf16 tensor with ld % 8 == 0")
    if out is None:
        out = torch.empty((rows + 63) // 64, dtype=torch.int64, device=dy.device)
    _chk(lib().mxr_rows_nonzero(_p(dy), rows, ld, _p(out), _s()), "rows_nonzero")
    return out


def rows_dilate(words: torch.Tensor, g: ConvGeom, nd: int = 1, out: Optional[torch.Tensor] = None) -> torch.Tensor:
    nw = (int(g.M) + 63) // 64
    if out is None:
        out = torch.empty((nd, nw), dtype=torch.int64, device=words.device)
    if not (words.numel() >= nw and out.is_contiguous() and tuple(out.shape) == (nd, nw)):
        raise RuntimeError("rows_dilate: mask sizes do not match the geometry")
    _chk(lib().mxr_rows_dilate(_p(words), _p(out), nd, nw, ctypes.byref(g), _s()), "rows_dilate")
    return out


def halo_active_tiles(tiles: torch.Tensor, ntiles: int, masks: torch.Tensor,
                      out: Optional[Tuple[torch.Tensor, torch.Tensor]] = None):
    k = int(masks.shape[0])
    if out is None:
        out = (torch.empty((k, ntiles), dtype=torch.int32, device=masks.device),
               torch.empty(k, dtype=torch.int32, device=masks.device))
    _chk(lib().mxr_halo_active_tiles(_p(tiles), ntiles, _p(masks), int(masks.shape[1]), k, _p(out[0]), _p(out[1]),
                                     _s()), "halo_active_tiles")
    return out


_WS: Dict[tuple, tuple] = {}


def _workspace(device, N: int, shapes, depth: int, nw: int, ntiles: int):
    key = (str(device), int(N), tuple(shapes), int(depth))
    ws = _WS.get(key)
    if ws is None:
        ws = (torch.zeros((depth + 1, nw), dtype=torch.int64, device=device),
              torch.zeros((depth + 1, ntiles), dtype=torch.int32, device=device),
              torch.zeros(depth + 1, dtype=torch.int32, device=device))
        _WS[key] = ws
    return ws


class GradChain:

    def __init__(self, depth: int):
        self.depth = int(depth)
        self.acts = None

    def start(self, dy: torch.Tensor, N: int, shapes: Sequence[Tuple[int, int]]) -> None:
        from .conv_launch import geom_pyramid
        self.acts = None
        ld = int(dy.shape[-1])
        if not (dy.is_cuda and dy.dtype == torch.bfloat16 and dy.is_contiguous() and ld % 8 == 0
                and 0 <= self.depth <= MAX_DEPTH):
            return
        shapes = tuple((int(h), int(w)) for h, w in shapes)
        g = geom_pyramid(N, shapes, 32, 32)
        if dy.numel() != int(g.M) * ld:
            return
        nw = (int(g.M) + 63) // 64
        tiles, nt = _hx.device_tiles(N, shapes, dy.device)
        masks, order, count = _workspace(dy.device, N, shapes, self.depth, nw, nt)
        rows_nonzero(dy, out=masks[0])
        if self.depth:
            rows_dilate(masks[0], g, self.depth, out=masks[1:])
        halo_active_tiles(tiles, nt, masks, out=(order, count))
        self.acts = [Activity(masks[k], order[k], count[k:k + 1], g.M, nt) for k in range(self.depth + 1)]

    def level(self, k: int) -> Optional[Activity]:
        if self.acts is None or not 0 <= k <= self.depth:
            return None
        return self.acts[k]
```

batchai_retinanet_horovod_coco_amd/train/engine.py:

```python
from __future__ import annotations

import contextlib
import os
from typing import Dict, Optional

import torch

from ..ops import anchors as anchor_ops
from ..ops import losses
from ..parallel import runtime
from ..parallel.distributed_optimizer import DistributedOptimizer
from .flat import FlatParams, backward_order
from .optimizer import KerasAdam, KerasSGD


_ROCTX = os.environ.get("MXR_ROCTX", "0") == "1"


class _range:

    def __init__(self, name: str):
        self.name = name

    def __enter__(self):
        if _ROCTX and torch.cuda.is_available():
            torch.cuda.nvtx.range_push(self.name)
        return self

    def __exit__(self, *a):
        if _ROCTX and torch.cuda.is_available():
            torch.cuda.nvtx.range_pop()


_PAD_FOCAL = os.environ.get("MXR_PAD_FOCAL", "1") == "1"

class Trainer:
    def __init__(self, model, lr: float = 1e-5, clipnorm: float = 0.001, compute_dtype: torch.dtype = torch.float32,
                 clip_mode: str = "local", compression=None, bucket_bytes: Optional[int] = None,
                 device: Optional[torch.device] = None, overlap: bool = True, target_backend: str = "auto",
                 optimizer: str = "adam", momentum: float = 0.0, nesterov: bool = False, weight_decay: float = 0.0,
                 ema_decay: float = 0.0, regression_loss: str = "smooth_l1", regression_weight: float = 1.0,
                 assigner: str = "iou", atss_topk: int = anchor_ops.ATSS_TOPK, classification_loss: str = "focal",
                 dfl_weight: float = losses.DFL_WEIGHT):
        from ..parallel.collectives import Compression
        self.regression_bins = int(getattr(model, "regression_bins", 0) or 0)
        self.regression_range = float(getattr(model, "regression_range", 8.0))
        if not self.regression_bins and dfl_weight != losses.DFL_WEIGHT:
            raise ValueError("dfl_weight goes with a distribution box head (regression_bins); this model has none")
        if not float(dfl_weight) >= 0:
            raise ValueError("dfl_weight must be >= 0, got {}".format(dfl_weight))
        self.dfl_weight = float(dfl_weight)
        if self.regression_bins:
            from ..ops import fp8 as _fp8
            if _fp8.enabled():
                raise ValueError("regression_bins={} does not go with fp8: the regression final's {} outputs would run "
                                 "in fp8".format(self.regression_bins, 4 * self.regression_bins * model.num_anchors))
        if classification_loss != "focal" and classification_loss not in losses.CLS_KINDS:
            raise ValueError("classification_loss must be 'focal' or one of {}, got {!r}".format(
                losses.CLS_KINDS, classification_loss))
        if classification_loss != "focal":
            from ..ops import fp8 as _fp8
            if _fp8.enabled():
                raise ValueError("classification_loss={!r} does not go with fp8: the classification final's focal loss "
                                 "is part of the fp8 epilogue".format(classification_loss))
        self.classification_loss = classification_loss
        if getattr(model, "head_norm", None) is not None:
            from ..ops import fp8 as _fp8
            if _fp8.enabled():
                raise ValueError("head_norm={!r} does not go with fp8: the fp8 tower layers hand fp8 copies of their "
                                 "ReLU outputs to each other".format(model.head_norm))
        if assigner not in ("iou", "atss"):
            raise ValueError("assigner must be 'iou' or 'atss', got {!r}".format(assigner))
        if assigner == "iou" and atss_topk != anchor_ops.ATSS_TOPK:
            raise ValueError("atss_topk goes with assigner='atss'; the fixed-threshold rule has no top-k")
        self.assigner = assigner
        self.atss_topk = anchor_ops._check_topk(atss_topk)
        if regression_loss != "smooth_l1" and regression_loss not in losses.IOU_KINDS:
            raise ValueError("regression_loss must be 'smooth_l1' or one of {}, got {!r}".format(
                losses.IOU_KINDS, regression_loss))
        if regression_loss == "smooth_l1" and regression_weight != 1.0:
            raise ValueError("regression_weight goes with the IoU regression losses; smooth_l1 has no weight")
        self.regression_loss = regression_loss
        self.regression_weight = float(regression_weight)
        self.device = device or (runtime.device() if runtime.is_initialized() else torch.device("cpu"))
        self.model = model.to(self.device)
        self.compute_dtype = compute_dtype
        self.flat = FlatParams(backward_order(self.model), device=self.device)
        if optimizer == "adam":
            if momentum or nesterov or weight_decay:
                raise ValueError("momentum, nesterov and weight_decay belong to optimizer='sgd'")
            self.base_optimizer = KerasAdam(self.flat, lr=lr, clipnorm=clipnorm, ema_decay=ema_decay)
        elif optimizer == "sgd":
            self.base_optimizer = KerasSGD(self.flat, lr=lr, momentum=momentum, nesterov=nesterov,
                                           weight_decay=weight_decay, clipnorm=clipnorm, ema_decay=ema_decay)
        else:
            raise ValueError("optimizer must be 'adam' or 'sgd', got {!r}".format(optimizer))
        self.optimizer = DistributedOptimizer(self.base_optimizer, compression=compression or Compression.none,
                                              clip_mode=clip_mode, bucket_bytes=bucket_bytes, overlap=overlap)
        if regression_loss != "smooth_l1":
            self.base_optimizer.regression_loss = regression_loss
            self.base_optimizer.regression_weight = self.regression_weight
        if classification_loss != "focal":
            self.base_optimizer.classification_loss = classification_loss
        if assigner != "iou":
            self.base_optimizer.assigner = assigner
            self.base_optimizer.atss_topk = self.atss_topk
        if self.dfl_weight != losses.DFL_WEIGHT:
            self.base_optimizer.dfl_weight = self.dfl_weight
        self.anchors = anchor_ops.AnchorCache()
        self.num_classes = model.num_classes
        self.target_backend = target_backend
        self.stop_training = False
        self.shapes_callback = None
        self.last_logs: Dict[str, torch.Tensor] = {}
        self.compute_weights = None
        self._ema_swapped = False
        from ..ops import native
        self._cls_pad_buf = native.ShapeSlots()
        self._focal_req = None
        self._reg_pad_buf = native.ShapeSlots()
        self.step_graphs = None
        from ..ops import fp8 as _fp8
        _fp8.reset_state()
        if (self.device.type == "cuda" and compute_dtype == torch.bfloat16 and native.available()
                and hasattr(self.model, "convs") and os.environ.get("MXR_NO_COMPUTE_WEIGHTS") != "1"):
            self.compute_weights = native.ComputeWeights(self.flat, self.model.convs())
            native.set_compute_weights(self.compute_weights)
        if self.device.type == "cuda" and native.available() and os.environ.get("MXR_NO_GRAD_SINKS") != "1":
            native.set_grad_sinks(native.GradSinks(self.flat, self.optimizer.notify_grad_ready))

    def compute_targets(self, images: torch.Tensor, gt: torch.Tensor, gt_count: torch.Tensor, image_hw: torch.Tensor):
        H, W = int(images.shape[1]), int(images.shape[2])
        anchors = self.anchors.get((H, W), self.device, self.shapes_callback)
        centers = self.anchors.centers((H, W), self.device, self.shapes_callback)
        from ..ops import native
        use_hip = (self.target_backend == "hip" or
                   (self.target_backend == "auto" and anchors.is_cuda and native.available()))
        if self.assigner == "atss":
            levels = self.anchors.levels((H, W), self.device, self.shapes_callback)
            if use_hip:
                return native.atss_targets(anchors, levels, gt, gt_count, image_hw, topk=self.atss_topk, centers=centers)
            state, label, reg = anchor_ops.atss_targets_torch(anchors, levels, gt, gt_count, image_hw,
                                                              topk=self.atss_topk, centers=centers)
            return state, label, reg, (state == 1).sum().to(torch.int32).reshape(1)
        if use_hip:
            return native.anchor_targets(anchors, gt, gt_count, image_hw, centers=centers)
        state, label, reg = anchor_ops.anchor_targets_torch(anchors, gt, gt_count, image_hw, centers=centers)
        return state, label, reg, (state == 1).sum().to(torch.int32).reshape(1)

    def _fused_losses(self) -> bool:
        from ..ops import native
        return self.device.type == "cuda" and native.available()

    def forward_backward(self, images, gt, gt_count, image_hw):
        with _range("targets"):
            state, label, reg_t, npos = self.compute_targets(images, gt, gt_count, image_hw)
        x = images.to(self.compute_dtype)
        req = self._focal_request(state, label, npos)
        if self.regression_bins and self._fused_losses():
            self.model.integral_request = state
        with _range("forward"):
            try:
                out = self.model(x)
            finally:
                if req is not None:
                    self.model.focal_request = None
                if self.regression_bins:
                    self.model.integral_request = None
        with _range("backward"):
            return self._losses_backward(out, reg_t, state, label, npos, self._loss_anchors(images))

    def _loss_anchors(self, images):
        if self.regression_loss == "smooth_l1" and self.classification_loss == "focal":
            return None
        return self.anchors.get((int(images.shape[1]), int(images.shape[2])), self.device, self.shapes_callback)

    def _regression_fwd_bwd(self, reg, reg_t, state, npos, anchors, **pad):
        from ..ops import native
        if self.regression_loss == "smooth_l1":
            return native.smooth_l1_fwd_bwd(reg, reg_t, state, npos, **pad)
        return native.iou_loss_fwd_bwd(reg, reg_t, anchors, state, npos, kind=self.regression_loss,
                                       weight=self.regression_weight, **pad)

    def _regression_torch(self, reg, reg_t, state, anchors):
        if self.regression_loss == "smooth_l1":
            return losses.smooth_l1_loss(reg, reg_t, state, backend="torch")
        return losses.iou_loss(reg, reg_t, state, anchors, self.regression_loss, self.regression_weight,
                               backend="torch")

    def _regression_terms_torch(self, out, reg_t, state, anchors):
        loss = self._regression_torch(out["regression"], reg_t, state, anchors)
        if self.regression_bins:
            loss = loss + losses.distribution_focal_loss(out["regression_logits"], reg_t, state, self.regression_bins,
                                                         self.regression_range, self.dfl_weight, backend="torch")
        return loss

    def _dist_losses_fused(self, out, reg_t, state, npos, anchors, A, rsink):
        from ..ops import native
        from ..ops import fp8 as _fp8
        if _fp8.enabled():
            raise RuntimeError("regression_bins={} does not go with fp8".format(self.regression_bins))
        K, R = self.regression_bins, self.regression_range
        logits, reg = out["regression_logits"], out["regression"]
        if reg.requires_grad:
            loss = self._regression_terms_torch(out, reg_t, state, anchors)
            return loss, loss, None
        box_loss, dreg = self._regression_fwd_bwd(reg, reg_t, state, npos, anchors)
        W = 4 * K * A
        if rsink is not None and _PAD_FOCAL and logits.dtype == torch.bfloat16 and logits.shape[1] % A == 0 and W % 64:
            key = (logits.shape[0], logits.shape[1] // A, (W + 63) // 64 * 64, logits.device)
            buf = self._reg_pad_buf.get(key, lambda: torch.zeros(key[:3], dtype=logits.dtype, device=logits.device))
            dfl, dpad = native.box_dist_fwd_bwd(logits.detach(), dreg, reg_t, state, npos, K, R, self.dfl_weight,
                                                grad_out=buf, group=A)
            rsink["dy"] = dpad
            dlog = torch.zeros((), dtype=logits.dtype, device=logits.device).expand(logits.shape)
        else:
            dfl, dlog = native.box_dist_fwd_bwd(logits.detach(), dreg, reg_t, state, npos, K, R, self.dfl_weight)
        return logits, box_loss + dfl, dlog

    def _check_quality_rows(self, cls, reg, anchors):
        if not (cls.dim() == 3 and reg.dim() == 3 and reg.shape[:2] == cls.shape[:2] and reg.shape[2] == 4
                and anchors is not None and anchors.shape[0] == cls.shape[1]):
            raise ValueError("classification_loss={!r} needs the regression output (B, A, 4) in the row order of the "
                             "classification output (B, A, C) and the A anchors of the batch's shape; got {} and {}"
                             .format(self.classification_loss, tuple(reg.shape), tuple(cls.shape)))

    def _classification_fwd_bwd(self, out, reg_t, state, label, npos, anchors, **pad):
        from ..ops import native
        cls = out["classification"]
        if getattr(self.model, "head_norm", None) is not None:
            from ..ops import fp8 as _fp8
            if _fp8.enabled():
                raise RuntimeError("head_norm={!r} does not go with fp8".format(self.model.head_norm))
        if self.classification_loss == "focal":
            return native.focal_fwd_bwd(cls, state, label, npos, **pad)
        from ..ops import fp8 as _fp8
        if _fp8.enabled():
            raise RuntimeError("classification_loss={!r} does not go with fp8".format(self.classification_loss))
        reg = out["regression"].detach()
        self._check_quality_rows(cls, reg, anchors)
        return native.quality_loss_fwd_bwd(cls, reg, reg_t, anchors, state, label, npos,
                                           kind=self.classification_loss, **pad)

    def _classification_torch(self, out, reg_t, state, label, anchors):
        cls = out["classification"]
        if self.classification_loss == "focal":
            return losses.focal_loss(cls, state, label, backend="torch")
        self._check_quality_rows(cls, out["regression"], anchors)
        return losses.quality_loss(cls, out["regression"], reg_t, state, label, anchors, self.classification_loss,
                                   backend="torch")

    def _focal_request(self, state, label, npos):
        if self.classification_loss != "focal":
            return None
        if not (self._fused_losses() and _PAD_FOCAL and self.compute_dtype == torch.bfloat16
                and hasattr(self.model, "cls_pad_sink")):
            return None
        from ..ops.conv_launch import FocalRequest
        if self._focal_req is None:
            self._focal_req = FocalRequest()
        A = self.model.num_anchors if hasattr(self.model, "num_anchors") else 9
        self._focal_req.set(state, label, npos, A)
        self.model.focal_request = self._focal_req
        return self._focal_req

    def _losses_backward(self, out, reg_t, state, label, npos, anchors=None):
        if self._fused_losses():
            from ..ops import native
            reg = out["regression"]
            A = self.model.num_anchors if hasattr(self.model, "num_anchors") else 9
            rsink = getattr(self.model, "reg_pad_sink", None)
            if self.regression_bins:
                reg, reg_loss, dreg = self._dist_losses_fused(out, reg_t, state, npos, anchors, A, rsink)
            elif rsink is not None and _PAD_FOCAL and reg.dtype == torch.bfloat16 and reg.shape[1] % A == 0 and \
                    (4 * A) % 64:
                key = (reg.shape[0], reg.shape[1] // A, (4 * A + 63) // 64 * 64, reg.device)
                buf = self._reg_pad_buf.get(key, lambda: torch.zeros(key[:3], dtype=reg.dtype, device=reg.device))
                reg_loss, dpad = self._regression_fwd_bwd(reg, reg_t, state, npos, anchors, grad_out=buf, group=A)
                rsink["dy"] = dpad
                dreg = torch.zeros((), dtype=reg.dtype, device=reg.device).expand(reg.shape)
            else:
                reg_loss, dreg = self._regression_fwd_bwd(reg, reg_t, state, npos, anchors)
            cls = out["classification"]
            sink = getattr(self.model, "cls_pad_sink", None)
            cp = (A * cls.shape[-1] + 63) // 64 * 64
            req = self._focal_req
            if req is not None and req.loss is not None:
                cls_loss = req.loss
                req.loss = None
                dcls = torch.zeros((), dtype=cls.dtype, device=cls.device).expand(cls.shape)
            elif sink is not None and _PAD_FOCAL and cls.dtype == torch.bfloat16 and cls.shape[1] % A == 0 and \
                    cls.shape[-1] % 8 == 0 and (A * cls.shape[-1]) % 64:
                key = (cls.shape[0], cls.shape[1] // A, cp, cls.device)
                buf = self._cls_pad_buf.get(key, lambda: torch.zeros(key[:3], dtype=cls.dtype, device=cls.device))
                cls_loss, dpad = self._classification_fwd_bwd(out, reg_t, state, label, npos, anchors, grad_out=buf,
                                                              group=A)
                sink["dy"] = dpad
                dcls = torch.zeros((), dtype=cls.dtype, device=cls.device).expand(cls.shape)
            else:
                cls_loss, dcls = self._classification_fwd_bwd(out, reg_t, state, label, npos, anchors)
            torch.autograd.backward([reg, cls], [dreg, dcls])
        else:
            reg_loss = self._regression_terms_torch(out, reg_t, state, anchors)
            cls_loss = self._classification_torch(out, reg_t, state, label, anchors)
            (reg_loss + cls_loss).backward()
        return reg_loss.detach(), cls_loss.detach()

    def forward_losses(self, images, gt, gt_count, image_hw):
        with torch.no_grad():
            state, label, reg_t, npos = self.compute_targets(images, gt, gt_count, image_hw)
            out = self.model(images.to(self.compute_dtype))
            anchors = self._loss_anchors(images)
            reg_loss = self._regression_terms_torch(out, reg_t, state, anchors)
            cls_loss = self._classification_torch(out, reg_t, state, label, anchors)
        return reg_loss, cls_loss

    def train_on_batch(self, images: torch.Tensor, gt: torch.Tensor, gt_count: torch.Tensor,
                       image_hw: torch.Tensor) -> Dict[str, torch.Tensor]:
        if not self.model.training:
            self.model.train()
        if self._ema_swapped:
# ... 138 lines not shown
```

csrc/kernels/conv_hx32.hip:

```cpp
#include <type_traits>

#include "common.h"
#include "conv_common.h"
#include "focal_common.h"
#include "halo_tile.h"

typedef __attribute__((ext_vector_type(16))) float f32x16;

namespace {

constexpr int H2_PLANE = HX_HMAX * 32;
constexpr int H2_HBYTES = 2 * H2_PLANE;
constexpr int H2_HPC = 2 * HX_HMAX / 32;

template <int N>
__device__ __forceinline__ void h2_vm_wait() {
  asm volatile("s_waitcnt vmcnt(%0)" ::"n"(N) : "memory");
}

__device__ __forceinline__ void h2_sync() {
  asm volatile("s_waitcnt lgkmcnt(0)" ::: "memory");
  __builtin_amdgcn_s_barrier();
  asm volatile("" ::: "memory");
}
// ... 164 lines not shown
      const int o = next ? hn[q] : hs[q];
      uintptr_t a = (o >= 0 && !(DIAG & 16)) ? (uintptr_t)(X + (long long)o + c * 32) : (uintptr_t)zpage;
      if constexpr ((DIAG & 32) != 0) a = (uintptr_t)(X + c * 16384 + k * 512 + lane * 8);
      glds16((const void*)a, dst);
    }
  };
  auto load_bias = [&](int co0) {
    float4 v = make_float4(0.f, 0.f, 0.f, 0.f);
    if (bias != nullptr && threadIdx.x < BCO / 4 && co0 + 4 * (int)threadIdx.x < cout)
      v = *reinterpret_cast<const float4*>(bias + co0 + 4 * threadIdx.x);
    return v;
  };
  auto store_bias = [&](int bb, float4 v) {
    if (threadIdx.x < BCO / 4) *reinterpret_cast<float4*>(smem + BOFF + bb * BCO * 4 + 16 * threadIdx.x) = v;
  };

  AccT acc[TI][TJ];

  auto stage = [&](auto kyc, auto slotc, auto bufc, auto&& dma) {
    constexpr int ky = decltype(kyc)::value, slot = decltype(slotc)::value, buf = decltype(bufc)::value;
    if constexpr (M16) {
      constexpr int TIH = TI / 2;
      static_assert(TJ % 2 == 0 && TI >= 2 && TI % 2 == 0, "M16 read schedule");
      int bq[TJ];
#pragma unroll
      for (int j = 0; j < TJ; ++j)
        bq[j] = HOFF + (HB1 ? 0 : buf) * H2_HBYTES + (lane >> 5) * H2_PLANE + (hb[j] + ky * hp[j]) * 32 +
                ((lane >> 4) & 1) * 16;
      const char* ws = smem + slot * STAGE + aoff;
      bf16x8 fa[3][TI], fb[3][TJ];
      auto rA = [&](auto kxc, auto ic) {
        constexpr int kx = decltype(kxc)::value, i = decltype(ic)::value;
        fa[kx][i] = *reinterpret_cast<const bf16x8*>(ws + kx * TAPB + i * 512);
      };
      auto rB = [&](auto kxc, auto jc) {
        constexpr int kx = decltype(kxc)::value, j = decltype(jc)::value;
        fb[kx][j] = *reinterpret_cast<const bf16x8*>(smem + bq[j] + kx * 32);
      };
      rA(std::integral_constant<int, 0>{}, std::integral_constant<int, 0>{});
      rA(std::integral_constant<int, 0>{}, std::integral_constant<int, 1>{});
      h2_for<0, TJ>([&](auto jc) { rB(std::integral_constant<int, 0>{}, jc); });
      __builtin_amdgcn_sched_group_barrier(0x0100, 2 + TJ, 0);
      h2_for<0, 6>([&](auto nc) {
        constexpr int n = decltype(nc)::value, kx = n >> 1, h = n & 1;
        constexpr int nd = decltype(dma(nc))::value;
        dma(nc);
        h2_for<0, TIH>([&](auto gc) {
          constexpr int g = decltype(gc)::value, i = h * TIH + g;
          constexpr bool ra = i + 2 < TI || kx + 1 < 3;
          constexpr int nb = (i >= TI - 2 && kx + 1 < 3) ? TJ / 2 : 0;
          if constexpr (i + 2 < TI) rA(std::integral_constant<int, kx>{}, std::integral_constant<int, i + 2>{});
          else if constexpr (kx + 1 < 3)
            rA(std::integral_constant<int, kx + 1>{}, std::integral_constant<int, i + 2 - TI>{});
          if constexpr (nb > 0)
            h2_for<0, nb>([&](auto bc) {
              rB(std::integral_constant<int, kx + 1>{},
                 std::integral_constant<int, (i - (TI - 2)) * (TJ / 2) + decltype(bc)::value>{});
            });
#pragma unroll
          for (int j = 0; j < TJ; ++j)
            acc[i][j] = __builtin_amdgcn_mfma_f32_16x16x32_bf16(fa[kx][i], fb[kx][j], acc[i][j], 0, 0, 0);
          constexpr int NRD = (ra ? 1 : 0) + nb;
          constexpr int NR = NRD < TJ ? NRD : TJ;
          h2_for<0, NR>([&](auto) {
            __builtin_amdgcn_sched_group_barrier(0x0008, 1, 0);
            __builtin_amdgcn_sched_group_barrier(0x0100, 1, 0);
          });
          if constexpr (NRD > NR) __builtin_amdgcn_sched_group_barrier(0x0100, NRD - NR, 0);
          constexpr int d0 = g * nd / TIH, d1 = (g + 1) * nd / TIH;
          constexpr int NM = TJ - NR;
          constexpr int NDG = d1 - d0 < NM ? d1 - d0 : NM;
          h2_for<0, NDG>([&](auto) {
            __builtin_amdgcn_sched_group_barrier(0x0008, 1, 0);
            __builtin_amdgcn_sched_group_barrier(0x0010, 1, 0);
          });
          if constexpr (d1 - d0 > NDG) __builtin_amdgcn_sched_group_barrier(0x0010, d1 - d0 - NDG, 0);
          if constexpr (NM > NDG) __builtin_amdgcn_sched_group_barrier(0x0008, NM - NDG, 0);
          __builtin_amdgcn_sched_barrier(0);
        });
      });
      return;
    } else {
    int ba[TJ][3][2];
#pragma unroll
    for (int j = 0; j < TJ; ++j)
#pragma unroll
      for (int kx = 0; kx < 3; ++kx) {
        const int h = hb[j] + ky * hp[j] + kx;
        if constexpr (HL) {
#pragma unroll
          for (int kh = 0; kh < 2; ++kh) ba[j][kx][kh] = HOFF + (HB1 ? 0 : buf) * H2_HBYTES + h * 64 + (((2 * kh + fh) ^ ((h >> 2) & 3)) << 4);
        } else {
          ba[j][kx][0] = HOFF + (HB1 ? 0 : buf) * H2_HBYTES + h2_off(h, fh);
          ba[j][kx][1] = ba[j][kx][0] + H2_PLANE;
        }
      }
    const char* ws = smem + slot * STAGE + aoff;
    auto rd = [&](auto nc, bf16x8* a, bf16x8* b) {
      constexpr int n = decltype(nc)::value, kx = n >> 1, kh = n & 1;
#pragma unroll
      for (int i = 0; i < TI; ++i) a[i] = *reinterpret_cast<const bf16x8*>(ws + kx * TAPB + kh * WPL + i * 1024);
#pragma unroll
      for (int j = 0; j < TJ; ++j) b[j] = *reinterpret_cast<const bf16x8*>(smem + ba[j][kx][kh]);
    };
    bf16x8 fa[2][TI], fb[2][TJ];
    rd(std::integral_constant<int, 0>{}, fa[0], fb[0]);
    __builtin_amdgcn_sched_group_barrier(0x0100, TI + TJ, 0);
    h2_for<0, 6>([&](auto nc) {
      constexpr int n = decltype(nc)::value;
      constexpr int nd = decltype(dma(nc))::value;
      dma(nc);
      if constexpr (n + 1 < 6) rd(std::integral_constant<int, n + 1>{}, fa[(n + 1) & 1], fb[(n + 1) & 1]);
#pragma unroll
      for (int i = 0; i < TI; ++i)
#pragma unroll
        for (int j = 0; j < TJ; ++j) {
          if constexpr ((DIAG & 64) != 0) {
            constexpr int o = (n & 1) * 8;
            f32x4 lo = {acc[i][j][o], acc[i][j][o + 1], acc[i][j][o + 2], acc[i][j][o + 3]};
            f32x4 hi = {acc[i][j][o + 4], acc[i][j][o + 5], acc[i][j][o + 6], acc[i][j][o + 7]};
            lo = __builtin_amdgcn_mfma_f32_16x16x32_bf16(fa[n & 1][i], fb[n & 1][j], lo, 0, 0, 0);
            hi = __builtin_amdgcn_mfma_f32_16x16x32_bf16(fa[n & 1][i], fb[n & 1][j], hi, 0, 0, 0);
#pragma unroll
            for (int e = 0; e < 4; ++e) { acc[i][j][o + e] = lo[e]; acc[i][j][o + 4 + e] = hi[e]; }
          } else {
            acc[i][j] = __builtin_amdgcn_mfma_f32_32x32x16_bf16(fa[n & 1][i], fb[n & 1][j], acc[i][j], 0, 0, 0);
          }
        }
      constexpr int MF = (DIAG & 64) ? 2 : 1;
      constexpr int NRD = n + 1 < 6 ? TI + TJ : 0;
      constexpr int NR = NRD < TI * TJ ? NRD : TI * TJ;
      h2_for<0, NR>([&](auto) {
        __builtin_amdgcn_sched_group_barrier(0x0008, MF, 0);
        __builtin_amdgcn_sched_group_barrier(0x0100, 1, 0);
      });
      if constexpr (NRD > NR) __builtin_amdgcn_sched_group_barrier(0x0100, NRD - NR, 0);
      constexpr int NM = TI * TJ - NR;
      constexpr int ND = nd < NM ? nd : NM;
      h2_for<0, ND>([&](auto) {
        __builtin_amdgcn_sched_group_barrier(0x0008, MF, 0);
        __builtin_amdgcn_sched_group_barrier(0x0010, 1, 0);
      });
      if constexpr (nd > ND) __builtin_amdgcn_sched_group_barrier(0x0010, nd - ND, 0);
      if constexpr (NM > ND) __builtin_amdgcn_sched_group_barrier(0x0008, MF * (NM - ND), 0);
    });
    }
  };

  int item = PERS ? (int)blockIdx.x : xcd_remap(blockIdx.x, gridDim.x);
  int nwork_c = nwork;
  if constexpr (ACT) {
    nwork_c = __builtin_amdgcn_readfirstlane(*act_cnt) * tiles_co;
    if constexpr (!PERS) item = (int)blockIdx.x < nwork_c ? xcd_remap(blockIdx.x, nwork_c) : (int)blockIdx.x;
    auto zero_item = [&](int z) {
      const HaloTile& T = tiles[tile_of(z)];
      const int zc0 = tile_co0(z);
      const int nchk = min(BCO, cout - zc0) >> 3;
      const int n = T.nslot * nchk;
      for (int i = threadIdx.x; i < n; i += NW * 64) {
        const int p = fdiv(i, nchk), ch = i - p * nchk;
        HX_SELECT(sbeg, p)
        int sb = T.b[0].sbeg, C = T.b[0].C, ob = T.b[0].out_base, W = T.b[0].W, y0 = T.b[0].y0, x0 = T.b[0].x0;
#pragma unroll
        for (int t = 1; t < HX_BOX; ++t)
          if (sel == t) {
            sb = T.b[t].sbeg; C = T.b[t].C; ob = T.b[t].out_base; W = T.b[t].W; y0 = T.b[t].y0; x0 = T.b[t].x0;
          }
        const int loc = p - sb;
        const int r = fdiv(loc, C), c = loc - r * C;
        *reinterpret_cast<uint4*>(Y + (long long)(ob + (y0 + r) * W + x0 + c) * cout + zc0 + ch * 8) =
            make_uint4(0u, 0u, 0u, 0u);
      }
    };
    if (!accumulate) {
      if constexpr (PERS) {
        for (int z = nwork_c + item; z < nwork; z += (int)gridDim.x) zero_item(z);
      } else if (item >= nwork_c) {
        zero_item(item);
      }
    }
    if (item >= nwork_c) return;
  }
  float foc_acc = 0.f, foc_inv = 0.f, foc_elo = 0.f, foc_ehi = 0.f;
  if constexpr (FOC > 0) {
    foc_inv = 1.0f / fmaxf(1.0f, (float)(*fa.npos));
    foc_elo = __expf(-fabsf(fa.lo));
    foc_ehi = __expf(-fabsf(fa.hi));
  }
  int co0 = tile_co0(item);
  int wvoff[NVO];
  w_voff(co0, wvoff);
  int hsrc[H2_HQ];
  decode_halo(item, hsrc);
  issue_halo(hsrc, hsrc, false, 0, 0, 0, H2_HQ);
  issue_w(wvoff, 0, 0, 0, 0, NWP);
  if constexpr (WR3) issue_w(wvoff, 1, 0, 1, 0, NWP);
  {
    const float4 bv4 = load_bias(co0);
    decode_frag(item);
    h2_vm_wait<0>();
    store_bias(0, bv4);
  }
  h2_sync();

  for (int bb = 0;; bb ^= 1) {
    const int nitem = item + (int)gridDim.x;
    const bool has_next = PERS && nitem < nwork_c;
    int nco0 = co0, nwvoff[NVO], nhsrc[H2_HQ];
#pragma unroll
    for (int v = 0; v < NVO; ++v) nwvoff[v] = wvoff[v];
#pragma unroll
    for (int q = 0; q < H2_HQ; ++q) nhsrc[q] = hsrc[q];
    if (has_next) {
      nco0 = tile_co0(nitem);
      w_voff(nco0, nwvoff);
      decode_halo(nitem, nhsrc);
    }
#pragma unroll
    for (int i = 0; i < TI; ++i)
#pragma unroll
      for (int j = 0; j < TJ; ++j)
#pragma unroll
        for (int e = 0; e < AE; ++e) acc[i][j][e] = 0.f;

    auto chunk = [&](int c, auto bufc) {
      constexpr int buf = decltype(bufc)::value;
      const bool more = c + 1 < nch;
      const bool chain = !more && has_next;
      const int cn = more ? c + 1 : (chain ? 0 : c);
      h2_for<0, 3>([&](auto kyc) {
        constexpr int ky = decltype(kyc)::value;
        constexpr int slot = WR3 ? ky : ((buf + ky) & 1);
        constexpr int wslot = WR3 ? (ky + 2) % 3 : (slot ^ 1);
        const int wky = WR3 ? (ky + 2) % 3 : (ky < 2 ? ky + 1 : 0);
        const int wc = WR3 ? (ky == 0 ? c : cn) : (ky < 2 ? c : cn);
        int wv[NVO];
#pragma unroll
        for (int v = 0; v < NVO; ++v) wv[v] = (ky == 2 && chain) ? nwvoff[v] : wvoff[v];
        auto dma = [&](auto nc) {
          constexpr int n = decltype(nc)::value;
          constexpr int m0 = n * WPS < NWP ? n * WPS : NWP, m1 = (n + 1) * WPS < NWP ? (n + 1) * WPS : NWP;
          if constexpr (m1 > m0) issue_w(wv, wky, wc, wslot, m0, m1);
          constexpr bool hs = ky == 0 && n >= 3 && n < 5 && !(DIAG & 2) && !HB1;
          constexpr int q0 = hs ? (n - 3) * HPS : 0, q1 = hs ? ((n - 2) * HPS < H2_HQ ? (n - 2) * HPS : H2_HQ) : 0;
          if constexpr (q1 > q0) issue_halo(hsrc, nhsrc, chain, cn, buf ^ 1, q0, q1);
          return std::integral_constant<int, (m1 - m0) + (q1 - q0)>{};
        };
        stage(kyc, std::integral_constant<int, slot>{}, bufc, dma);
        if (ky < 2 || more) {
          if constexpr (WR3) {
            if constexpr (ky < 2) h2_vm_wait<NWP + H2_HQ>();
            else h2_vm_wait<NWP>();
          } else if constexpr (ky == 0 && !HB1) h2_vm_wait<(DIAG & 2) ? 0 : H2_HQ>();
          else h2_vm_wait<0>();
          h2_sync();
          if constexpr (HB1 && ky == 2) {
            issue_halo(hsrc, nhsrc, false, cn, 0, 0, H2_HQ);
            h2_vm_wait<0>();
            h2_sync();
          }
        }
      });
    };
    for (int c = 0; c < nch; c += 2) {
      chunk(c, std::integral_constant<int, 0>{});
      if (c + 1 < nch) chunk(c + 1, std::integral_constant<int, 1>{});
    }

    if constexpr (DIAG & 8) {
      float sacc = 0.f;
#pragma unroll
      for (int i = 0; i < TI; ++i)
#pragma unroll
        for (int j = 0; j < TJ; ++j) sacc += acc[i][j][0] + acc[i][j][AE - 1];
      if (sacc == 1234.5f) Y[threadIdx.x] = 0;
    } else {
      const bf16_t* Yacc = (MK || FOC || BW) ? nullptr : (accumulate ? Y : nullptr);
      const bf16_t* Rs_ = (MK || FOC || BW) ? nullptr : Rs;
      const bf16_t* Mk_ = (MK || FOC || BW) ? nullptr : Mk;
      const bool plain = Rs_ == nullptr && Yacc == nullptr && Mk_ == nullptr;
      auto put8 = [&](uint4 o, int off, int cg, int mo_, uint32_t mb, uint4 m) {
        if (plain) {
          if constexpr (MK == 2) {
            o.x &= h2_keep2(mb, 0); o.y &= h2_keep2(mb, 1); o.z &= h2_keep2(mb, 2); o.w &= h2_keep2(mb, 3);
          } else if constexpr (MK != 0) {
            o.x = h2_mask2(o.x, m.x); o.y = h2_mask2(o.y, m.y); o.z = h2_mask2(o.z, m.z); o.w = h2_mask2(o.w, m.w);
          }
          if (!MK && relu) {
            o.x = h2_relu2(o.x); o.y = h2_relu2(o.y); o.z = h2_relu2(o.z); o.w = h2_relu2(o.w);
          }
          if constexpr (BW != 0) mkb[off >> 3] = (uint8_t)h2_bits8(o);
        } else {
          const uint32_t w4[4] = {o.x, o.y, o.z, o.w};
          float v[8];
#pragma unroll
          for (int e = 0; e < 4; ++e) {
            v[2 * e] = bf2f((bf16_t)(w4[e] & 0xffff));
            v[2 * e + 1] = bf2f((bf16_t)(w4[e] >> 16));
          }
          epi_sweep8(v, Rs_, off, Yacc, Mk_, off, relu);
          o.x = (uint32_t)f2bf(v[0]) | ((uint32_t)f2bf(v[1]) << 16);
          o.y = (uint32_t)f2bf(v[2]) | ((uint32_t)f2bf(v[3]) << 16);
          o.z = (uint32_t)f2bf(v[4]) | ((uint32_t)f2bf(v[5]) << 16);
          o.w = (uint32_t)f2bf(v[6]) | ((uint32_t)f2bf(v[7]) << 16);
        }
        if constexpr (FOC > 0) {
          const int pix = mo_ / cout;
          const int a = cg / FOC, c0 = cg - a * FOC;
          const long long row = (long long)pix * fa.A + a;
          const int st = fa.state[row];
          float gv[8];
          if (st == -1) {
#pragma unroll
            for (int e = 0; e < 8; ++e) gv[e] = 0.f;
          } else {
            const int lb = st == 1 ? fa.label[row] - c0 : -1;
            const uint32_t w4[4] = {o.x, o.y, o.z, o.w};
            float v[8];
#pragma unroll
            for (int e = 0; e < 4; ++e) {
              v[2 * e] = bf2f((bf16_t)(w4[e] & 0xffff));
              v[2 * e + 1] = bf2f((bf16_t)(w4[e] >> 16));
            }
            foc_acc += focal8_g2(v, lb, fa.alpha, fa.gamma, fa.lo, fa.hi, foc_elo, foc_ehi, foc_inv, gv);
// ... 70 lines not shown
                mw[j][qp] = make_uint4(0u, 0u, 0u, 0u);
                if (mo[j] >= 0 && cg < cout) mw[j][qp] = *reinterpret_cast<const uint4*>(Mk + mo[j] + cg);
              }
            }
        }
        float4 bv[4];
#pragma unroll
        for (int q = 0; q < 4; ++q)
          bv[q] = *reinterpret_cast<const float4*>(smem + BOFF + bb * BCO * 4 +
                                                   4 * (wco * WT_CO + i * 32 + 8 * q + 4 * fh));
#pragma unroll
        for (int j = 0; j < TJ; ++j) {
          uint32_t pk[4][2];
#pragma unroll
          for (int q = 0; q < 4; ++q) {
            pk[q][0] = (uint32_t)f2bf(acc[i][j][4 * q] + bv[q].x) | ((uint32_t)f2bf(acc[i][j][4 * q + 1] + bv[q].y) << 16);
            pk[q][1] = (uint32_t)f2bf(acc[i][j][4 * q + 2] + bv[q].z) | ((uint32_t)f2bf(acc[i][j][4 * q + 3] + bv[q].w) << 16);
          }
#pragma unroll
          for (int qp = 0; qp < 2; ++qp)
#pragma unroll
            for (int d = 0; d < 2; ++d) {
              const auto r = __builtin_amdgcn_permlane32_swap(pk[2 * qp][d], pk[2 * qp + 1][d], false, false);
              pk[2 * qp][d] = r[0];
              pk[2 * qp + 1][d] = r[1];
            }
#pragma unroll
          for (int qp = 0; qp < 2; ++qp) {
            const int cg = co0 + wco * WT_CO + i * 32 + 16 * qp + 8 * fh;
            if (mo[j] < 0 || cg >= cout) continue;
            put8(make_uint4(pk[2 * qp][0], pk[2 * qp][1], pk[2 * qp + 1][0], pk[2 * qp + 1][1]), mo[j] + cg, cg, mo[j],
                 MK == 2 ? mbyte[j][qp] : 0u, MK == 1 ? mw[j][qp] : make_uint4(0u, 0u, 0u, 0u));
          }
        }
      }
      }
    }
    if (!has_next) break;
    item = nitem;
    co0 = nco0;
#pragma unroll
    for (int v = 0; v < NVO; ++v) wvoff[v] = nwvoff[v];
#pragma unroll
    for (int q = 0; q < H2_HQ; ++q) hsrc[q] = nhsrc[q];
    const float4 bv4 = load_bias(co0);
    decode_frag(item);
    h2_vm_wait<0>();
    store_bias(bb ^ 1, bv4);
    h2_sync();
  }
  h2_vm_wait<0>();
  if constexpr (FOC > 0) {
    __shared__ float fred[16];
    const float bs = block_sum(foc_acc, fred);
    if (threadIdx.x == 0) fa.partials[blockIdx.x] = bs;
  }
}

template <int BCO, int PERS, int DIAG = 0, int HL = 0, int NWV = 8, int HB1 = 0, int WR3 = 0, int MK = 0, int FOC = 0,
          int BW = 0, int M16 = 0, int ACT = 0>
int launch_hx32(const bf16_t* X, const bf16_t* Wt, const float* bias, const bf16_t* R, const bf16_t* Mk, bf16_t* Y,
                const bf16_t* zpage, const HaloTile* tiles, int ntiles, const ConvGeom& g, int relu, int accumulate,
                hipStream_t stream, const FocalArgs& fa = FocalArgs{}, const int* act_list = nullptr,
                const int* act_cnt = nullptr) {
  const int tiles_co = (g.cout + BCO - 1) / BCO;
  const long long nwork = (long long)tiles_co * ntiles;
  if (nwork > 0x7fffffffLL || nwork < 1) return -3;
  if (PERS && (g.cin / 32) % 2 != 0) return -5;
  const size_t lds = (size_t)(WR3 ? 9 : 6) * BCO * 64 + (HB1 ? 1 : 2) * (size_t)H2_HBYTES + 2 * BCO * 4;
  auto kern = conv3x3_hx32_kernel<BCO, PERS, DIAG, HL, NWV, HB1, WR3, MK, FOC, BW, M16, ACT>;
  static bool attr_set = false;
  static int ncu = 0;
  if (!attr_set) {
    hipFuncSetAttribute((const void*)kern, hipFuncAttributeMaxDynamicSharedMemorySize, (int)lds);
    int dev = 0;
    hipGetDevice(&dev);
    hipDeviceGetAttribute(&ncu, hipDeviceAttributeMultiprocessorCount, dev);
    if (ncu < 1) ncu = 256;
    attr_set = true;
  }
  const long long grid = PERS ? std::min<long long>(nwork, ncu) : nwork;
  kern<<<(unsigned)grid, NWV * 64, lds, stream>>>(X, Wt, bias, R, Mk, Y, zpage, tiles, g, relu, accumulate, tiles_co,
                                                    (int)nwork, fa, act_list, act_cnt);
  return (int)hipGetLastError();
}

__global__ void hx32_pack_kernel(const uint4* __restrict__ W, uint4* __restrict__ Wp, int cout, int cin, long long n) {
  const long long i = (long long)blockIdx.x * blockDim.x + threadIdx.x;
  if (i >= n) return;
  const int h = (int)(i & 1);
  long long r = i >> 1;
  const int co = (int)(r % cout);
  r /= cout;
  const int p = (int)(r & 1);
  r >>= 1;
  const int nch = cin >> 5;
  const int c = (int)(r % nch);
  const int tap = (int)(r / nch);
  Wp[i] = W[((long long)co * 9 + tap) * (cin >> 3) + c * 4 + p * 2 + h];
}

struct PackSeg {
  long long src;
  long long doff;
  long long ustart;
  int cout, cin;
};

__global__ void hx32_pack_batch_kernel(const PackSeg* __restrict__ segs, int nseg, uint4* __restrict__ dst,
                                       long long total) {
  const long long i = (long long)blockIdx.x * blockDim.x + threadIdx.x;
  if (i >= total) return;
  int lo = 0, hi = nseg - 1;
  while (lo < hi) {
    const int mid = (lo + hi + 1) >> 1;
    if (segs[mid].ustart <= i) lo = mid; else hi = mid - 1;
  }
  const PackSeg s = segs[lo];
  const long long u = i - s.ustart;
  const int h = (int)(u & 1);
  long long r = u >> 1;
  const int co = (int)(r % s.cout);
  r /= s.cout;
  const int p = (int)(r & 1);
  r >>= 1;
  const int nch = s.cin >> 5;
  const int c = (int)(r % nch);
  const int tap = (int)(r / nch);
  const uint4* W = reinterpret_cast<const uint4*>(s.src);
  dst[s.doff / 8 + u] = W[((long long)co * 9 + tap) * (s.cin >> 3) + c * 4 + p * 2 + h];
}

}

MXR_API int mxr_hx32_pack_batch(const void* segs, int nseg, void* dst, long long total_units, hipStream_t stream) {
  if (nseg < 1 || total_units < 1) return -1;
  const long long nb = (total_units + 255) / 256;
  if (nb > 0x7fffffffLL) return -2;
  hx32_pack_batch_kernel<<<(unsigned)nb, 256, 0, stream>>>((const PackSeg*)segs, nseg, (uint4*)dst, total_units);
  return (int)hipGetLastError();
}

MXR_API int mxr_hx32_pack_weights(const void* W, void* Wp, int cout, int cin, hipStream_t stream) {
  if (cin % 32 != 0 || cout < 1) return -1;
  const long long n = (long long)cout * 9 * cin / 8;
  hx32_pack_kernel<<<(unsigned)((n + 255) / 256), 256, 0, stream>>>((const uint4*)W, (uint4*)Wp, cout, cin, n);
  return (int)hipGetLastError();
}

namespace {

#define HX_LAUNCH(...)                                                                                            \
  launch_hx32<__VA_ARGS__, ACT>(x, w, bias, r, mk, y, z, t, ntiles, g, relu, accumulate, stream, FocalArgs{}, al, ac)

template <int ACT>
int hx32_dispatch(const bf16_t* x, const bf16_t* w, const float* bias, const bf16_t* r, const bf16_t* mk, bf16_t* y,
                  const bf16_t* z, const HaloTile* t, int ntiles, const ConvGeom& g, int relu, int accumulate,
                  int variant, hipStream_t stream, const int* al, const int* ac) {
  const bool bits = mk != nullptr && ((uintptr_t)mk & 1);
  const bool mk_fast = mk != nullptr && r == nullptr && !accumulate && !relu;
  if (mk_fast && variant == 0 && !bits) return HX_LAUNCH(256, 0, 0, 0, 8, 0, 0, 1, 0, 0, 0);
  if (mk_fast && variant == 6 && !bits) return HX_LAUNCH(128, 0, 0, 0, 8, 1, 0, 1, 0, 0, 0);
  if (mk_fast && variant == 0 && bits) return HX_LAUNCH(256, 0, 0, 0, 8, 0, 0, 2, 0, 0, 0);
  if (mk_fast && variant == 6 && bits) return HX_LAUNCH(128, 0, 0, 0, 8, 1, 0, 2, 0, 0, 0);
  if (mk_fast && variant == 10 && !bits) return HX_LAUNCH(256, 0, 0, 0, 8, 0, 0, 1, 0, 0, 1);
  if (mk_fast && variant == 10 && bits) return HX_LAUNCH(256, 0, 0, 0, 8, 0, 0, 2, 0, 0, 1);
  if (mk_fast && variant == 11 && !bits) return HX_LAUNCH(128, 0, 0, 0, 8, 1, 0, 1, 0, 0, 1);
  if (mk_fast && variant == 11 && bits) return HX_LAUNCH(128, 0, 0, 0, 8, 1, 0, 2, 0, 0, 1);
  if constexpr (!ACT) {
    const bool bw_fast = bits && relu && r == nullptr && !accumulate;
    if (bw_fast && variant == 0) return HX_LAUNCH(256, 0, 0, 0, 8, 0, 0, 0, 0, 1, 0);
    if (bw_fast && variant == 6) return HX_LAUNCH(128, 0, 0, 0, 8, 1, 0, 0, 0, 1, 0);
    if (bw_fast && variant == 10) return HX_LAUNCH(256, 0, 0, 0, 8, 0, 0, 0, 0, 1, 1);
    if (bw_fast && variant == 11) return HX_LAUNCH(128, 0, 0, 0, 8, 1, 0, 0, 0, 1, 1);
  }
  switch (variant) {
    case 0: return HX_LAUNCH(256, 0, 0, 0, 8, 0, 0, 0, 0, 0, 0);
    case 1: return HX_LAUNCH(128, 0, 0, 0, 8, 0, 0, 0, 0, 0, 0);
    case 2: return HX_LAUNCH(256, 1, 0, 0, 8, 0, 0, 0, 0, 0, 0);
    case 3: return HX_LAUNCH(128, 1, 0, 0, 8, 0, 0, 0, 0, 0, 0);
    case 4: return HX_LAUNCH(256, 0, 0, 1, 8, 0, 0, 0, 0, 0, 0);
    case 5: return HX_LAUNCH(128, 0, 0, 1, 8, 0, 0, 0, 0, 0, 0);
    case 6: return HX_LAUNCH(128, 0, 0, 0, 8, 1, 0, 0, 0, 0, 0);
    case 7: return HX_LAUNCH(128, 0, 0, 0, 8, 0, 1, 0, 0, 0, 0);
    case 8: return HX_LAUNCH(64, 0, 0, 0, 4, 0, 0, 0, 0, 0, 0);
    case 9: return HX_LAUNCH(64, 0, 0, 0, 4, 1, 0, 0, 0, 0, 0);
    case 10: return HX_LAUNCH(256, 0, 0, 0, 8, 0, 0, 0, 0, 0, 1);
    case 11: return HX_LAUNCH(128, 0, 0, 0, 8, 1, 0, 0, 0, 0, 1);
    case 12: return HX_LAUNCH(128, 0, 0, 0, 8, 0, 0, 0, 0, 0, 1);
    case 13: return HX_LAUNCH(256, 1, 0, 0, 8, 0, 0, 0, 0, 0, 1);
    case 14: return HX_LAUNCH(128, 1, 0, 0, 8, 0, 0, 0, 0, 0, 1);
    case 15: return HX_LAUNCH(128, 0, 0, 0, 8, 0, 1, 0, 0, 0, 1);
    default: break;
  }
#ifdef MXR_DIAG_KERNELS
  if constexpr (!ACT) {
    switch (variant) {
      case 101: return HX_LAUNCH(256, 1, 1, 0, 8, 0, 0, 0, 0, 0, 0);
      case 102: return HX_LAUNCH(256, 1, 2, 0, 8, 0, 0, 0, 0, 0, 0);
      case 103: return HX_LAUNCH(256, 1, 3, 0, 8, 0, 0, 0, 0, 0, 0);
      case 108: return HX_LAUNCH(256, 1, 8, 0, 8, 0, 0, 0, 0, 0, 0);
      case 111: return HX_LAUNCH(256, 1, 11, 0, 8, 0, 0, 0, 0, 0, 0);
      case 132: return HX_LAUNCH(256, 0, 32, 0, 8, 0, 0, 0, 0, 0, 0);
      case 116: return HX_LAUNCH(256, 0, 16, 0, 8, 0, 0, 0, 0, 0, 0);
      case 126: return HX_LAUNCH(128, 0, 16, 0, 8, 1, 0, 0, 0, 0, 0);
      case 164: return HX_LAUNCH(256, 0, 64, 0, 8, 0, 0, 0, 0, 0, 0);
      case 170: return HX_LAUNCH(128, 0, 64, 0, 8, 1, 0, 0, 0, 0, 0);
      default: break;
    }
  }
#endif
  return -6;
}
#undef HX_LAUNCH

}

MXR_API int mxr_conv3x3_hx32_act(const void* X, const void* Wt, const float* bias, const void* R, const void* Mk,
                                 void* Y, const void* zpage, const ConvGeom* g, const void* tiles, int ntiles, int relu,
                                 int accumulate, int variant, const int* act_list, const int* act_cnt,
                                 hipStream_t stream) {
  if (g->cin % 32 != 0 || g->cout % 8 != 0) return -1;
  if (g->kh != 3 || g->kw != 3 || g->stride != 1 || g->pt != 1 || g->pl != 1 || g->ostride != 1) return -2;
  if (g->in_img != g->out_img || (g->M + 1) * (long long)std::max(g->cin, g->cout) >= (1LL << 31)) return -4;
  if ((long long)g->cout * 9 * g->cin * 2 >= (1LL << 31)) return -4;
  const bf16_t *x = (const bf16_t*)X, *w = (const bf16_t*)Wt, *r = (const bf16_t*)R, *mk = (const bf16_t*)Mk;
  const bf16_t* z = (const bf16_t*)zpage;
  const HaloTile* t = (const HaloTile*)tiles;
  bf16_t* y = (bf16_t*)Y;
  if ((act_list == nullptr) != (act_cnt == nullptr)) return -7;
  if (act_list != nullptr) {
    if (bias != nullptr || r != nullptr || relu) return -7;
    return hx32_dispatch<1>(x, w, bias, r, mk, y, z, t, ntiles, *g, relu, accumulate, variant, stream, act_list,
                            act_cnt);
  }
  return hx32_dispatch<0>(x, w, bias, r, mk, y, z, t, ntiles, *g, relu, accumulate, variant, stream, nullptr, nullptr);
}

MXR_API int mxr_conv3x3_hx32(const void* X, const void* Wt, const float* bias, const void* R, const void* Mk,
                             void* Y, const void* zpage, const ConvGeom* g, const void* tiles, int ntiles, int relu,
                             int accumulate, int variant, hipStream_t stream) {
  return mxr_conv3x3_hx32_act(X, Wt, bias, R, Mk, Y, zpage, g, tiles, ntiles, relu, accumulate, variant, nullptr,
                              nullptr, stream);
}

void mxr_loss_finalize_launch(const float* partials, int n, const int* npos, float* out, hipStream_t stream);

MXR_API int mxr_conv3x3_hx32_focal_v(const void* X, const void* Wt, const float* bias, const void* zpage,
                                     const ConvGeom* g, const void* tiles, int ntiles, const int8_t* state,
                                     const int32_t* label, const int* npos, void* dpad, int ld, int A, int C, float alpha,
                                     float gamma, float lo, float hi, float* partials, int nparts, float* out, int variant,
                                     hipStream_t stream) {
  if (g->cin % 32 != 0 || g->cout % 8 != 0) return -1;
  if (g->kh != 3 || g->kw != 3 || g->stride != 1 || g->pt != 1 || g->pl != 1 || g->ostride != 1) return -2;
  if (g->in_img != g->out_img || (g->M + 1) * (long long)std::max(g->cin, g->cout) >= (1LL << 31)) return -4;
  if ((long long)g->cout * 9 * g->cin * 2 >= (1LL << 31)) return -4;
  if (C != 80 || gamma != 2.0f || A * C != g->cout || ld < g->cout || ld % 8 != 0) return -8;
  const long long nwork = (long long)((g->cout + 255) / 256) * ntiles;
  if (nparts < nwork || (long long)g->M * ld >= (1LL << 31)) return -9;
  const FocalArgs fa{state, label, npos, (bf16_t*)dpad, partials, ld, A, alpha, gamma, lo, hi};
  if (variant != 0 && variant != 10) return -6;
  const int rc =
      variant == 10
          ? launch_hx32<256, 0, 0, 0, 8, 0, 0, 0, 80, 0, 1>((const bf16_t*)X, (const bf16_t*)Wt, bias, nullptr, nullptr,
                                                            nullptr, (const bf16_t*)zpage, (const HaloTile*)tiles,
                                                            ntiles, *g, 0, 0, stream, fa)
          : launch_hx32<256, 0, 0, 0, 8, 0, 0, 0, 80>((const bf16_t*)X, (const bf16_t*)Wt, bias, nullptr, nullptr,
                                                      nullptr, (const bf16_t*)zpage, (const HaloTile*)tiles,
                                                      ntiles, *g, 0, 0, stream, fa);
  if (rc) return rc;
  mxr_loss_finalize_launch(partials, (int)nwork, npos, out, stream);
  return (int)hipGetLastError();
}

MXR_API int mxr_conv3x3_hx32_focal(const void* X, const void* Wt, const float* bias, const void* zpage,
                                   const ConvGeom* g, const void* tiles, int ntiles, const int8_t* state,
                                   const int32_t* label, const int* npos, void* dpad, int ld, int A, int C, float alpha,
                                   float gamma, float lo, float hi, float* partials, int nparts, float* out,
                                   hipStream_t stream) {
  return mxr_conv3x3_hx32_focal_v(X, Wt, bias, zpage, g, tiles, ntiles, state, label, npos, dpad, ld, A, C, alpha, gamma,
                                  lo, hi, partials, nparts, out, 0, stream);
}
```

csrc/kernels/row_activity.hip:

```cpp
#include "common.h"
#include "conv_common.h"
#include "halo_tile.h"

typedef unsigned long long u64;

namespace {

__global__ __launch_bounds__(256) void rows_nonzero_kernel(const uint4* __restrict__ dy, long long rows, int cpr,
                                                           u64* __restrict__ mask) {
  __shared__ unsigned int bits[2];
  if (threadIdx.x < 2) bits[threadIdx.x] = 0u;
  __syncthreads();
  const long long r0 = (long long)blockIdx.x * 64;
  const int nr = (int)(rows - r0 < 64 ? rows - r0 : 64);
  const int n = nr * cpr;
  const uint4* src = dy + r0 * cpr;
  for (int c = threadIdx.x; c < n; c += 256) {
    const uint4 v = src[c];
    if (((v.x | v.y | v.z | v.w) & 0x7fff7fffu) != 0u) {
      const int r = c / cpr;
      atomicOr(&bits[r >> 5], 1u << (r & 31));
    }
  }
  __syncthreads();
  if (threadIdx.x == 0) mask[blockIdx.x] = (u64)bits[0] | ((u64)bits[1] << 32);
}

__device__ __forceinline__ u64 ra_bits(const u64* __restrict__ mask, long long nw, long long s, int len) {
  const long long w = s >> 6;
  const int o = (int)(s & 63);
  u64 v = mask[w] >> o;
  if (o + len > 64 && w + 1 < nw) v |= mask[w + 1] << (64 - o);
  return v & ((1ull << len) - 1ull);
}

constexpr int RA_MAXD = 8;

__global__ __launch_bounds__(256) void rows_dilate_kernel(const u64* __restrict__ in, u64* __restrict__ out, int nd,
                                                          long long stride, long long nw, ConvGeom g) {
  const long long m = (long long)blockIdx.x * 256 + threadIdx.x;
  int dmin = 2 * RA_MAXD;
  if (m < g.M) {
    const int b = (int)(m / g.out_img);
    const int q = (int)(m - (long long)b * g.out_img);
    LevelSel s;
    select_level(g, q, s);
    const int loc = q - s.mstart;
    const int y = loc / s.wo, x = loc - y * s.wo;
    const long long base = (long long)b * g.out_img + s.mstart;
    const int xa = max(0, x - nd), xb = min(s.W - 1, x + nd);
    const int cx = x - xa;
    for (int dy = -nd; dy <= nd; ++dy) {
      const int yy = y + dy;
      if ((unsigned)yy >= (unsigned)s.H) continue;
      const u64 w = ra_bits(in, nw, base + (long long)yy * s.W + xa, xb - xa + 1);
      if (w == 0ull) continue;
      int dh = 2 * RA_MAXD;
      const u64 lo = w & ((2ull << cx) - 1ull);
      if (lo) dh = cx - (63 - __builtin_clzll(lo));
      const u64 hi = w >> cx;
      if (hi) dh = min(dh, (int)__builtin_ctzll(hi));
      dmin = min(dmin, max(dh, dy < 0 ? -dy : dy));
    }
  }
  const long long word = m >> 6;
  for (int k = 1; k <= nd; ++k) {
    const u64 bal = __ballot(dmin <= k);
    if ((threadIdx.x & 63) == 0 && word < nw) out[(long long)(k - 1) * stride + word] = bal;
  }
}

__device__ __forceinline__ bool ra_tile_active(const HaloTile& T, const u64* __restrict__ mask) {
  for (int b = 0; b < T.nbox; ++b) {
    const HaloBox& B = T.b[b];
    const int ya = max(0, B.y0 - 1), yb = min(B.H - 1, B.y0 + B.R);
    const int xa = max(0, B.x0 - 1), xb = min(B.W - 1, B.x0 + B.C);
    for (int yy = ya; yy <= yb; ++yy) {
      long long s = (long long)B.out_base + (long long)yy * B.W + xa;
      int len = xb - xa + 1;
      while (len > 0) {
        const int o = (int)(s & 63);
        const int n = min(64 - o, len);
        const u64 v = (mask[s >> 6] >> o) & (n == 64 ? ~0ull : ((1ull << n) - 1ull));
        if (v) return true;
        s += n;
        len -= n;
      }
    }
  }
  return false;
}

__global__ __launch_bounds__(1024) void halo_active_tiles_kernel(const HaloTile* __restrict__ tiles, int ntiles,
                                                                 const u64* __restrict__ masks, long long stride,
                                                                 int* __restrict__ lists, int* __restrict__ counts) {
  __shared__ int wcnt[16];
  __shared__ int base_s;
  const u64* mask = masks + (long long)blockIdx.x * stride;
  int* list = lists + (long long)blockIdx.x * ntiles;
  const int lane = threadIdx.x & 63, wave = threadIdx.x >> 6;
  if (threadIdx.x == 0) base_s = 0;
  __syncthreads();
  for (int t0 = 0; t0 < ntiles; t0 += 1024) {
    const int t = t0 + threadIdx.x;
    const bool act = t < ntiles && ra_tile_active(tiles[t], mask);
    const u64 bal = __ballot(act);
    if (lane == 0) wcnt[wave] = __popcll(bal);
    __syncthreads();
    int before = base_s;
    for (int w = 0; w < wave; ++w) before += wcnt[w];
    const int rank = before + __popcll(bal & ((1ull << lane) - 1ull));
    if (t < ntiles) {
      if (act) list[rank] = t;
      else list[ntiles - 1 - (t - rank)] = t;
    }
    __syncthreads();
    if (threadIdx.x == 0) {
      int s = base_s;
      for (int w = 0; w < 16; ++w) s += wcnt[w];
      base_s = s;
    }
    __syncthreads();
  }
  if (threadIdx.x == 0) counts[blockIdx.x] = base_s;
}

}

MXR_API int mxr_rows_nonzero(const void* dy, long long rows, int ld, void* mask, hipStream_t stream) {
  if (rows < 1 || ld < 8 || ld % 8 != 0 || ((uintptr_t)dy & 15)) return -1;
  const long long nw = (rows + 63) / 64;
  if (nw > 0x7fffffffLL) return -4;
  rows_nonzero_kernel<<<(unsigned)nw, 256, 0, stream>>>((const uint4*)dy, rows, ld / 8, (u64*)mask);
  return (int)hipGetLastError();
}

MXR_API int mxr_rows_dilate(const void* in, void* out, int nd, long long stride_words, const ConvGeom* g,
                            hipStream_t stream) {
  if (nd < 1 || nd > RA_MAXD || g->nlev < 1 || g->nlev > MXR_MAXLEV || g->M < 1) return -1;
  const long long nw = (g->M + 63) / 64;
  if (stride_words < nw || nw > 0x7fffffffLL) return -4;
  for (int l = 0; l < g->nlev; ++l)
    if (g->W[l] != g->Wo[l] || g->H[l] != g->Ho[l]) return -2;
  rows_dilate_kernel<<<(unsigned)((nw + 3) / 4), 256, 0, stream>>>((const u64*)in, (u64*)out, nd, stride_words, nw, *g);
  return (int)hipGetLastError();
}

MXR_API int mxr_halo_active_tiles(const void* tiles, int ntiles, const void* masks, long long stride_words, int nmask,
                                  int* lists, int* counts, hipStream_t stream) {
  if (ntiles < 1 || nmask < 1) return -1;
  halo_active_tiles_kernel<<<(unsigned)nmask, 1024, 0, stream>>>((const HaloTile*)tiles, ntiles, (const u64*)masks,
                                                                 stride_words, lists, counts);
  return (int)hipGetLastError();
}
```

Before: 567.6 images/sec.

## Skip forward regression-head conv tiles outside positive-anchor receptive fields

```diff
diff --git a/batchai_retinanet_horovod_coco_amd/models/retinanet.py b/batchai_retinanet_horovod_coco_amd/models/retinanet.py
--- a/batchai_retinanet_horovod_coco_amd/models/retinanet.py
+++ b/batchai_retinanet_horovod_coco_amd/models/retinanet.py
@@ -89,7 +89,7 @@
         w, b = self.final.effective(x[0].dtype)
         return conv_ops.pyramid_conv(x, w, b, relu=False)
 
-    def forward_packed(self, x: torch.Tensor, shapes, pad_sink=None, join=None, chain=None) -> torch.Tensor:
+    def forward_packed(self, x: torch.Tensor, shapes, pad_sink=None, join=None, chain=None, fwd=None) -> torch.Tensor:
         from ..ops import native_conv
         from ..ops import fp8
         if self.norms is not None:
@@ -107,9 +107,11 @@
             x = native_conv.pyramid_conv_layer(x, shapes, c, True, mask_input_grad=i > 0, grad_premasked=True,
                                                join=join if i == 0 else None,
                                                out_f8=fp8.eligible(nxt.cin, nxt.cout),
-                                               act=None if chain is None else (chain, len(self.tower) - i))
+                                               act=None if chain is None else (chain, len(self.tower) - i),
+                                               need=None if fwd is None else fwd.need(len(self.tower) - i))
         return native_conv.pyramid_conv_layer(x, shapes, self.final, False, mask_input_grad=True,
-                                              pad_sink=pad_sink, act=None if chain is None else (chain, 0))
+                                              pad_sink=pad_sink, act=None if chain is None else (chain, 0),
+                                              need=None if fwd is None else fwd.need(0))
 
     def convs(self) -> List[Conv2D]:
         return list(self.tower) + [self.final]
@@ -174,11 +176,20 @@
                                                os.environ.get("MXR_GRAD_JOIN", "1") == "1") else None
             self.reg_pad_sink = {} if torch.is_grad_enabled() else None
             from ..ops import fp8, row_activity
-            chain = None
-            if (torch.is_grad_enabled() and row_activity.enabled() and packed.dtype == torch.bfloat16
-                    and self.head_norm is None and not fp8.enabled()):
-                chain = row_activity.GradChain(len(self.regression_submodel.tower))
-            reg = self.regression_submodel.forward_packed(packed, shapes, self.reg_pad_sink, join=join, chain=chain)
+            chain = fwd = None
+            if (torch.is_grad_enabled() and packed.dtype == torch.bfloat16 and self.head_norm is None
+                    and not fp8.enabled()):
+                depth = len(self.regression_submodel.tower)
+                state = getattr(self, "positive_request", None)
+                if state is not None and row_activity.fwd_enabled():
+                    fwd = row_activity.FwdChain(depth)
+                    fwd.start(state, self.num_anchors, B, shapes)
+                    if fwd.acts is None:
+                        fwd = None
+                if row_activity.enabled():
+                    chain = row_activity.GradChain(depth, fwd=fwd)
+            reg = self.regression_submodel.forward_packed(packed, shapes, self.reg_pad_sink, join=join, chain=chain,
+                                                          fwd=fwd)
             self.cls_pad_sink = {} if torch.is_grad_enabled() else None
             req = getattr(self, "focal_request", None)
             if self.cls_pad_sink is not None and req is not None:
diff --git a/batchai_retinanet_horovod_coco_amd/ops/conv_launch.py b/batchai_retinanet_horovod_coco_amd/ops/conv_launch.py
--- a/batchai_retinanet_horovod_coco_amd/ops/conv_launch.py
+++ b/batchai_retinanet_horovod_coco_amd/ops/conv_launch.py
@@ -244,7 +244,13 @@
     tiles, nt = _hx.device_tiles(_hx.geom_batch(g), _hx.geom_shapes(g), x.device)
     wp = hx32_packed(w, g.cout, g.cin)
     act = active if active is not None else _ra.current()
-    if act is not None and act.M == int(g.M) and act.ntiles == nt and bias is None and res is None and not relu:
+    fits = act is not None and act.M == int(g.M) and act.ntiles == nt
+    if fits and act.need and res is None and not accumulate and (mask is None or (relu and isinstance(mask, BitMask))):
+        _ra.FWD_LAUNCHES["conv"] += 1
+        return _chk(lib().mxr_conv3x3_hx32_need(_p(x), _p(wp), _p(bias), _p(mask), _p(y), _p(zero_page(x.device)),
+                                                ctypes.byref(g), _p(tiles), nt, int(relu), int(variant),
+                                                _p(act.order), _p(act.count), _s()), "conv3x3_hx32_need")
+    if fits and not act.need and bias is None and res is None and not relu:
         _ra.LAUNCHES["dgrad"] += 1
         return _chk(lib().mxr_conv3x3_hx32_act(_p(x), _p(wp), None, None, _p(mask), _p(y), _p(zero_page(x.device)),
                                                ctypes.byref(g), _p(tiles), nt, 0, int(accumulate), int(variant),
diff --git a/batchai_retinanet_horovod_coco_amd/ops/halo.py b/batchai_retinanet_horovod_coco_amd/ops/halo.py
--- a/batchai_retinanet_horovod_coco_amd/ops/halo.py
+++ b/batchai_retinanet_horovod_coco_amd/ops/halo.py
@@ -161,12 +161,16 @@
     return out
 
 
-def active_tiles(tab: np.ndarray, rows: np.ndarray) -> np.ndarray:
+def rows_positive(state: np.ndarray, group: int) -> np.ndarray:
+    return (np.asarray(state).reshape(-1, int(group)) == 1).any(axis=1)
+
+
+def active_tiles(tab: np.ndarray, rows: np.ndarray, ext: int = 1) -> np.ndarray:
     act = np.zeros(len(tab), dtype=bool)
     for i, row in enumerate(tab):
         for (sbeg, hoff, ib, ob, H, W, y0, x0, R, C) in _boxes(row):
-            ya, yb = max(0, y0 - 1), min(H - 1, y0 + R)
-            xa, xb = max(0, x0 - 1), min(W - 1, x0 + C)
+            ya, yb = max(0, y0 - ext), min(H - 1, y0 + R - 1 + ext)
+            xa, xb = max(0, x0 - ext), min(W - 1, x0 + C - 1 + ext)
             lv = rows[ob:ob + H * W].reshape(H, W)
             if lv[ya:yb + 1, xa:xb + 1].any():
                 act[i] = True
diff --git a/batchai_retinanet_horovod_coco_amd/ops/native.py b/batchai_retinanet_horovod_coco_amd/ops/native.py
--- a/batchai_retinanet_horovod_coco_amd/ops/native.py
+++ b/batchai_retinanet_horovod_coco_amd/ops/native.py
@@ -116,6 +116,10 @@
     "mxr_rows_nonzero": [c_vp, c_ll, c_int, c_vp, c_vp],
     "mxr_rows_dilate": [c_vp, c_vp, c_int, c_ll, ctypes.POINTER(ConvGeom), c_vp],
     "mxr_halo_active_tiles": [c_vp, c_int, c_vp, c_ll, c_int, c_vp, c_vp, c_vp],
+    "mxr_rows_positive": [c_vp, c_ll, c_int, c_vp, c_vp],
+    "mxr_halo_active_tiles_ext": [c_vp, c_int, c_vp, c_ll, c_int, c_int, c_vp, c_vp, c_vp, c_vp, c_vp],
+    "mxr_conv3x3_hx32_need": [c_vp, c_vp, c_vp, c_vp, c_vp, c_vp, ctypes.POINTER(ConvGeom), c_vp, c_int, c_int, c_int,
+                              c_vp, c_vp, c_vp],
     "mxr_conv_wgrad_pipe": [c_vp, c_vp, c_int, c_vp, c_int, c_vp, c_vp, c_int, c_vp, ctypes.POINTER(ConvGeom), c_int,
                             c_vp],
     "mxr_conv_wgrad_pipe_direct": [c_vp, c_vp, c_int, c_vp, c_vp, c_int, c_vp, ctypes.POINTER(ConvGeom), c_int, c_vp],
diff --git a/batchai_retinanet_horovod_coco_amd/ops/native_conv.py b/batchai_retinanet_horovod_coco_amd/ops/native_conv.py
--- a/batchai_retinanet_horovod_coco_amd/ops/native_conv.py
+++ b/batchai_retinanet_horovod_coco_amd/ops/native_conv.py
@@ -310,7 +310,7 @@
 
     @staticmethod
     def forward(ctx, x, weight, bias, shapes, relu, mask_input_grad=False, grad_premasked=False, pad_sink=None,
-                join=None, out_f8=False, act=None):
+                join=None, out_f8=False, act=None, need=None):
         from .conv_tuner import TUNER
         ctx.act = act
         x = x.contiguous()
@@ -357,8 +357,10 @@
             cands = fwd_candidates(x, w, b, None, g, 1, (1, 1, 1, 1), relu, (N, P, cout), allow_miopen=False,
                                    mask=emit)
             if cout % 8 and cout < 64:
-                cands["pad64"] = lambda: _pad64_pfwd(x, w, b, shapes, relu)
-            y = TUNER.run(key, cands)
+                cands["pad64"] = lambda: _pad64_pfwd(x, w, b, shapes, relu, need=nact)
+            nact = need if need is not None and not TUNER.needs_tuning(key, cands) else None
+            with _ra.using(nact):
+                y = TUNER.run(key, cands)
             if emit is not None:
                 y._mxr_bits = emit
         ctx.save_for_backward(x, w, y if relu else None)
@@ -465,7 +467,7 @@
                     dw = dw.to(ctx.wdt)
                 if has_bias and ctx.needs_input_grad[2] and not fb:
                     db = deliver_bias_grad(ctx.params[1], dy, channels=cout)
-                return dx, dw, db, None, None, None, None, None, None, None, None
+                return dx, dw, db, None, None, None, None, None, None, None, None, None
             with _ra.using(wact):
                 fused_bias = (has_bias and ctx.needs_input_grad[2]
                               and deliver_wgrad_bias_fused(wkey, x, dy, gw, ctx.params[0], ctx.params[1]))
@@ -497,7 +499,7 @@
                 dw = dw.to(ctx.wdt)
         if has_bias and ctx.needs_input_grad[2] and not fused_bias:
             db = deliver_bias_grad(ctx.params[1], dy, channels=cout)
-        return dx, dw, db, None, None, None, None, None, None, None, None
+        return dx, dw, db, None, None, None, None, None, None, None, None, None
 
 def _focal_fused(pad_sink, relu, b, g: ConvGeom, key: str) -> bool:
     from . import conv_launch as _cl
@@ -507,15 +509,17 @@
             and req.A > 0 and g.cout == 80 * req.A and _cl.hx32_covers(g)
             and (TUNER.prefer(key, "hx32_10", _cl.FOCAL_PREFER_MS) or TUNER.prefer(key, "hx32_0", _cl.FOCAL_PREFER_MS)))
 
-def _pad64_pfwd(x, w, b, shapes, relu):
+def _pad64_pfwd(x, w, b, shapes, relu, need=None):
     from .conv_tuner import TUNER
     N, P, cin = x.shape
     cout = w.shape[0]
     wp = F.pad(w, (0, 0, 0, 0, 0, 0, 0, 64 - cout)).contiguous()
     bp = None if b is None else F.pad(b, (0, 64 - cout)).contiguous()
     gp = geom_pyramid(N, shapes, cin, 64)
-    yp = TUNER.run(TUNER.key("pfwd", N, tuple(shapes), cin, 64, int(relu), "pad"),
-                   fwd_candidates(x, wp, bp, None, gp, 1, (1, 1, 1, 1), relu, (N, P, 64), allow_miopen=False))
+    key = TUNER.key("pfwd", N, tuple(shapes), cin, 64, int(relu), "pad")
+    cands = fwd_candidates(x, wp, bp, None, gp, 1, (1, 1, 1, 1), relu, (N, P, 64), allow_miopen=False)
+    with _ra.using(need if need is not None and not TUNER.needs_tuning(key, cands) else None):
+        yp = TUNER.run(key, cands)
     return yp[..., :cout].contiguous()
 
 def _pad64_pwgrad(x, dy, shapes, cout):
@@ -601,9 +605,9 @@
     return packed, shapes
 
 def pyramid_conv_layer(x, shapes, layer, relu, mask_input_grad=False, grad_premasked=False,
-                       pad_sink=None, join=None, out_f8: bool = False, act=None) -> torch.Tensor:
+                       pad_sink=None, join=None, out_f8: bool = False, act=None, need=None) -> torch.Tensor:
     return PyramidConvFn.apply(x, layer.weight, layer.bias, tuple(shapes), bool(relu), bool(mask_input_grad),
-                               bool(grad_premasked), pad_sink, join, bool(out_f8), act)
+                               bool(grad_premasked), pad_sink, join, bool(out_f8), act, need)
 
 def pyramid_unpack(y, shapes):
     out, off = [], 0
diff --git a/batchai_retinanet_horovod_coco_amd/ops/row_activity.py b/batchai_retinanet_horovod_coco_amd/ops/row_activity.py
--- a/batchai_retinanet_horovod_coco_amd/ops/row_activity.py
+++ b/batchai_retinanet_horovod_coco_amd/ops/row_activity.py
@@ -11,17 +11,24 @@
 
 MAX_DEPTH = 8
 LAUNCHES = {"dgrad": 0, "wgrad": 0}
+FWD_LAUNCHES = {"conv": 0}
+MASK_LAUNCHES = {"fwd": 0, "bwd": 0}
 
 
 def enabled() -> bool:
     return os.environ.get("MXR_SPARSE_REG_GRAD", "1") == "1"
 
 
+def fwd_enabled() -> bool:
+    return os.environ.get("MXR_SPARSE_REG_FWD", "1") != "0"
+
+
 class Activity:
-    __slots__ = ("words", "order", "count", "M", "ntiles")
-
-    def __init__(self, words, order, count, M, ntiles):
+    __slots__ = ("words", "order", "count", "M", "ntiles", "need")
+
+    def __init__(self, words, order, count, M, ntiles, need=False):
         self.words, self.order, self.count, self.M, self.ntiles = words, order, count, int(M), int(ntiles)
+        self.need = bool(need)
 
 
 _CUR = [None]
@@ -67,40 +74,123 @@
     return out
 
 
+def rows_positive(state: torch.Tensor, rows: int, group: int, out: Optional[torch.Tensor] = None) -> torch.Tensor:
+    rows, group = int(rows), int(group)
+    if not (state.is_cuda and state.dtype == torch.int8 and state.is_contiguous() and rows >= 1 and group >= 1
+            and state.numel() == rows * group):
+        raise RuntimeError("rows_positive: a contiguous int8 state of rows * group anchors")
+    nw = (rows + 63) // 64
+    if out is None:
+        out = torch.empty(nw, dtype=torch.int64, device=state.device)
+    if not (out.is_contiguous() and out.numel() >= nw and out.dtype == torch.int64):
+        raise RuntimeError("rows_positive: the mask does not hold the rows")
+    _chk(lib().mxr_rows_positive(_p(state), rows, group, _p(out), _s()), "rows_positive")
+    return out
+
+
 def halo_active_tiles(tiles: torch.Tensor, ntiles: int, masks: torch.Tensor,
-                      out: Optional[Tuple[torch.Tensor, torch.Tensor]] = None):
+                      out: Optional[Tuple[torch.Tensor, torch.Tensor]] = None,
+                      which: Optional[Sequence[int]] = None, ext: Optional[Sequence[int]] = None):
     k = int(masks.shape[0])
-    if out is None:
-        out = (torch.empty((k, ntiles), dtype=torch.int32, device=masks.device),
-               torch.empty(k, dtype=torch.int32, device=masks.device))
-    _chk(lib().mxr_halo_active_tiles(_p(tiles), ntiles, _p(masks), int(masks.shape[1]), k, _p(out[0]), _p(out[1]),
-                                     _s()), "halo_active_tiles")
+    if (which is None) != (ext is None):
+        raise RuntimeError("halo_active_tiles: which and ext go together")
+    nl = k if which is None else len(which)
+    if which is not None and not (len(ext) == nl and 1 <= nl <= 16 and all(0 <= int(w) < k for w in which)
+                                  and all(int(e) in (0, 1) for e in ext)):
+        raise RuntimeError("halo_active_tiles: which / ext do not match the masks")
+    if out is None:
+        out = (torch.empty((nl, ntiles), dtype=torch.int32, device=masks.device),
+               torch.empty(nl, dtype=torch.int32, device=masks.device))
+    if not (out[0].is_contiguous() and out[0].numel() >= nl * ntiles and out[1].numel() >= nl):
+        raise RuntimeError("halo_active_tiles: the lists do not hold the tiles")
+    if which is None:
+        _chk(lib().mxr_halo_active_tiles(_p(tiles), ntiles, _p(masks), int(masks.shape[1]), k, _p(out[0]), _p(out[1]),
+                                         _s()), "halo_active_tiles")
+    else:
+        wa = (ctypes.c_int * nl)(*[int(w) for w in which])
+        ea = (ctypes.c_int * nl)(*[int(e) for e in ext])
+        _chk(lib().mxr_halo_active_tiles_ext(_p(tiles), ntiles, _p(masks), int(masks.shape[1]), k, nl,
+                                             ctypes.cast(wa, ctypes.c_void_p), ctypes.cast(ea, ctypes.c_void_p),
+                                             _p(out[0]), _p(out[1]), _s()), "halo_active_tiles_ext")
     return out
 
 
 _WS: Dict[tuple, tuple] = {}
 
 
-def _workspace(device, N: int, shapes, depth: int, nw: int, ntiles: int):
-    key = (str(device), int(N), tuple(shapes), int(depth))
+_GEN: Dict[tuple, int] = {}
+
+
+def _workspace(device, N: int, shapes, depth: int, nw: int, ntiles: int, fwd: bool = False):
+    key = (str(device), int(N), tuple(shapes), int(depth), bool(fwd))
     ws = _WS.get(key)
     if ws is None:
+        nl = depth + 2 if fwd else depth + 1
         ws = (torch.zeros((depth + 1, nw), dtype=torch.int64, device=device),
-              torch.zeros((depth + 1, ntiles), dtype=torch.int32, device=device),
-              torch.zeros(depth + 1, dtype=torch.int32, device=device))
+              torch.zeros((nl, ntiles), dtype=torch.int32, device=device),
+              torch.zeros(nl, dtype=torch.int32, device=device))
         _WS[key] = ws
-    return ws
-
-
-class GradChain:
+    return ws + (key,) if fwd else ws
+
+
+class FwdChain:
 
     def __init__(self, depth: int):
         self.depth = int(depth)
         self.acts = None
+        self.gacts = None
+        self.geom = None
+        self._key = self._gen = None
+
+    def start(self, state: torch.Tensor, group: int, N: int, shapes: Sequence[Tuple[int, int]]) -> None:
+        from .conv_launch import geom_pyramid
+        self.acts = self.gacts = None
+        shapes = tuple((int(h), int(w)) for h, w in shapes)
+        g = geom_pyramid(N, shapes, 32, 32)
+        M, d = int(g.M), self.depth
+        if not (state is not None and state.is_cuda and state.dtype == torch.int8 and state.is_contiguous()
+                and int(group) >= 1 and state.numel() == M * int(group) and 0 <= d <= MAX_DEPTH):
+            return
+        nw = (M + 63) // 64
+        tiles, nt = _hx.device_tiles(N, shapes, state.device)
+        masks, order, count, key = _workspace(state.device, N, shapes, d, nw, nt, fwd=True)
+        rows_positive(state, M, group, out=masks[0])
+        if d:
+            rows_dilate(masks[0], g, d, out=masks[1:])
+        halo_active_tiles(tiles, nt, masks, out=(order, count), which=list(range(d + 1)) + [0], ext=[1] * (d + 1) + [0])
+        MASK_LAUNCHES["fwd"] += 3 if d else 2
+        self._key = key
+        self._gen = _GEN[key] = _GEN.get(key, 0) + 1
+        self.geom = (int(N), shapes)
+        lst = [d + 1] + list(range(d))
+        self.acts = [Activity(masks[k], order[lst[k]], count[lst[k]:lst[k] + 1], M, nt, need=True)
+                     for k in range(d + 1)]
+        self.gacts = [Activity(masks[k], order[k], count[k:k + 1], M, nt) for k in range(d + 1)]
+
+    def current(self) -> bool:
+        return self.acts is not None and _GEN.get(self._key) == self._gen
+
+    def need(self, k: int) -> Optional[Activity]:
+        if self.acts is None or not 0 <= k <= self.depth:
+            return None
+        return self.acts[k]
+
+
+class GradChain:
+
+    def __init__(self, depth: int, fwd: Optional[FwdChain] = None):
+        self.depth = int(depth)
+        self.acts = None
+        self.fwd = fwd
 
     def start(self, dy: torch.Tensor, N: int, shapes: Sequence[Tuple[int, int]]) -> None:
         from .conv_launch import geom_pyramid
         self.acts = None
+        f = self.fwd
+        if (f is not None and f.depth == self.depth and f.current()
+                and f.geom == (int(N), tuple((int(h), int(w)) for h, w in shapes))):
+            self.acts = f.gacts
+            return
         ld = int(dy.shape[-1])
         if not (dy.is_cuda and dy.dtype == torch.bfloat16 and dy.is_contiguous() and ld % 8 == 0
                 and 0 <= self.depth <= MAX_DEPTH):
@@ -116,6 +206,7 @@
         if self.depth:
             rows_dilate(masks[0], g, self.depth, out=masks[1:])
         halo_active_tiles(tiles, nt, masks, out=(order, count))
+        MASK_LAUNCHES["bwd"] += 3 if self.depth else 2
         self.acts = [Activity(masks[k], order[k], count[k:k + 1], g.M, nt) for k in range(self.depth + 1)]
 
     def level(self, k: int) -> Optional[Activity]:
diff --git a/batchai_retinanet_horovod_coco_amd/train/engine.py b/batchai_retinanet_horovod_coco_amd/train/engine.py
--- a/batchai_retinanet_horovod_coco_amd/train/engine.py
+++ b/batchai_retinanet_horovod_coco_amd/train/engine.py
@@ -159,6 +159,10 @@
         req = self._focal_request(state, label, npos)
         if self.regression_bins and self._fused_losses():
             self.model.integral_request = state
+        sparse_reg = (self._fused_losses() and self.classification_loss == "focal" and not self.regression_bins
+                      and self.regression_loss in ("smooth_l1", "giou", "diou", "ciou"))
+        if sparse_reg:
+            self.model.positive_request = state
         with _range("forward"):
             try:
                 out = self.model(x)
@@ -167,6 +171,8 @@
                     self.model.focal_request = None
                 if self.regression_bins:
                     self.model.integral_request = None
+                if sparse_reg:
+                    self.model.positive_request = None
         with _range("backward"):
             return self._losses_backward(out, reg_t, state, label, npos, self._loss_anchors(images))
 
diff --git a/csrc/kernels/conv_hx32.hip b/csrc/kernels/conv_hx32.hip
--- a/csrc/kernels/conv_hx32.hip
+++ b/csrc/kernels/conv_hx32.hip
@@ -340,6 +340,7 @@
   if constexpr (ACT) {
     nwork_c = __builtin_amdgcn_readfirstlane(*act_cnt) * tiles_co;
     if constexpr (!PERS) item = (int)blockIdx.x < nwork_c ? xcd_remap(blockIdx.x, nwork_c) : (int)blockIdx.x;
+    const bool zbits = ACT == 2 && relu && ((uintptr_t)Mk & 1);
     auto zero_item = [&](int z) {
       const HaloTile& T = tiles[tile_of(z)];
       const int zc0 = tile_co0(z);
@@ -356,8 +357,11 @@
           }
         const int loc = p - sb;
         const int r = fdiv(loc, C), c = loc - r * C;
-        *reinterpret_cast<uint4*>(Y + (long long)(ob + (y0 + r) * W + x0 + c) * cout + zc0 + ch * 8) =
-            make_uint4(0u, 0u, 0u, 0u);
+        const long long zoff = (long long)(ob + (y0 + r) * W + x0 + c) * cout + zc0 + ch * 8;
+        *reinterpret_cast<uint4*>(Y + zoff) = make_uint4(0u, 0u, 0u, 0u);
+        if constexpr (ACT == 2) {
+          if (zbits) mkb[zoff >> 3] = (uint8_t)0;
+        }
       }
     };
     if (!accumulate) {
@@ -734,22 +738,27 @@
 
 #define HX_LAUNCH(...)                                                                                            \
   launch_hx32<__VA_ARGS__, ACT>(x, w, bias, r, mk, y, z, t, ntiles, g, relu, accumulate, stream, FocalArgs{}, al, ac)
+#define HX_LAUNCH_G(...)                                                                                          \
+  launch_hx32<__VA_ARGS__, (ACT == 2 ? 3 : ACT)>(x, w, bias, r, mk, y, z, t, ntiles, g, relu, accumulate, stream,    \
+                                                 FocalArgs{}, al, ac)
 
 template <int ACT>
 int hx32_dispatch(const bf16_t* x, const bf16_t* w, const float* bias, const bf16_t* r, const bf16_t* mk, bf16_t* y,
                   const bf16_t* z, const HaloTile* t, int ntiles, const ConvGeom& g, int relu, int accumulate,
                   int variant, hipStream_t stream, const int* al, const int* ac) {
   const bool bits = mk != nullptr && ((uintptr_t)mk & 1);
-  const bool mk_fast = mk != nullptr && r == nullptr && !accumulate && !relu;
-  if (mk_fast && variant == 0 && !bits) return HX_LAUNCH(256, 0, 0, 0, 8, 0, 0, 1, 0, 0, 0);
-  if (mk_fast && variant == 6 && !bits) return HX_LAUNCH(128, 0, 0, 0, 8, 1, 0, 1, 0, 0, 0);
-  if (mk_fast && variant == 0 && bits) return HX_LAUNCH(256, 0, 0, 0, 8, 0, 0, 2, 0, 0, 0);
-  if (mk_fast && variant == 6 && bits) return HX_LAUNCH(128, 0, 0, 0, 8, 1, 0, 2, 0, 0, 0);
-  if (mk_fast && variant == 10 && !bits) return HX_LAUNCH(256, 0, 0, 0, 8, 0, 0, 1, 0, 0, 1);
-  if (mk_fast && variant == 10 && bits) return HX_LAUNCH(256, 0, 0, 0, 8, 0, 0, 2, 0, 0, 1);
-  if (mk_fast && variant == 11 && !bits) return HX_LAUNCH(128, 0, 0, 0, 8, 1, 0, 1, 0, 0, 1);
-  if (mk_fast && variant == 11 && bits) return HX_LAUNCH(128, 0, 0, 0, 8, 1, 0, 2, 0, 0, 1);
-  if constexpr (!ACT) {
+  if constexpr (ACT != 2) {
+    const bool mk_fast = mk != nullptr && r == nullptr && !accumulate && !relu;
+    if (mk_fast && variant == 0 && !bits) return HX_LAUNCH(256, 0, 0, 0, 8, 0, 0, 1, 0, 0, 0);
+    if (mk_fast && variant == 6 && !bits) return HX_LAUNCH(128, 0, 0, 0, 8, 1, 0, 1, 0, 0, 0);
+    if (mk_fast && variant == 0 && bits) return HX_LAUNCH(256, 0, 0, 0, 8, 0, 0, 2, 0, 0, 0);
+    if (mk_fast && variant == 6 && bits) return HX_LAUNCH(128, 0, 0, 0, 8, 1, 0, 2, 0, 0, 0);
+    if (mk_fast && variant == 10 && !bits) return HX_LAUNCH(256, 0, 0, 0, 8, 0, 0, 1, 0, 0, 1);
+    if (mk_fast && variant == 10 && bits) return HX_LAUNCH(256, 0, 0, 0, 8, 0, 0, 2, 0, 0, 1);
+    if (mk_fast && variant == 11 && !bits) return HX_LAUNCH(128, 0, 0, 0, 8, 1, 0, 1, 0, 0, 1);
+    if (mk_fast && variant == 11 && bits) return HX_LAUNCH(128, 0, 0, 0, 8, 1, 0, 2, 0, 0, 1);
+  }
+  if constexpr (ACT != 1) {
     const bool bw_fast = bits && relu && r == nullptr && !accumulate;
     if (bw_fast && variant == 0) return HX_LAUNCH(256, 0, 0, 0, 8, 0, 0, 0, 0, 1, 0);
     if (bw_fast && variant == 6) return HX_LAUNCH(128, 0, 0, 0, 8, 1, 0, 0, 0, 1, 0);
@@ -757,18 +766,18 @@
     if (bw_fast && variant == 11) return HX_LAUNCH(128, 0, 0, 0, 8, 1, 0, 0, 0, 1, 1);
   }
   switch (variant) {
-    case 0: return HX_LAUNCH(256, 0, 0, 0, 8, 0, 0, 0, 0, 0, 0);
+    case 0: return HX_LAUNCH_G(256, 0, 0, 0, 8, 0, 0, 0, 0, 0, 0);
     case 1: return HX_LAUNCH(128, 0, 0, 0, 8, 0, 0, 0, 0, 0, 0);
     case 2: return HX_LAUNCH(256, 1, 0, 0, 8, 0, 0, 0, 0, 0, 0);
     case 3: return HX_LAUNCH(128, 1, 0, 0, 8, 0, 0, 0, 0, 0, 0);
     case 4: return HX_LAUNCH(256, 0, 0, 1, 8, 0, 0, 0, 0, 0, 0);
     case 5: return HX_LAUNCH(128, 0, 0, 1, 8, 0, 0, 0, 0, 0, 0);
-    case 6: return HX_LAUNCH(128, 0, 0, 0, 8, 1, 0, 0, 0, 0, 0);
+    case 6: return HX_LAUNCH_G(128, 0, 0, 0, 8, 1, 0, 0, 0, 0, 0);
     case 7: return HX_LAUNCH(128, 0, 0, 0, 8, 0, 1, 0, 0, 0, 0);
     case 8: return HX_LAUNCH(64, 0, 0, 0, 4, 0, 0, 0, 0, 0, 0);
     case 9: return HX_LAUNCH(64, 0, 0, 0, 4, 1, 0, 0, 0, 0, 0);
-    case 10: return HX_LAUNCH(256, 0, 0, 0, 8, 0, 0, 0, 0, 0, 1);
-    case 11: return HX_LAUNCH(128, 0, 0, 0, 8, 1, 0, 0, 0, 0, 1);
+    case 10: return HX_LAUNCH_G(256, 0, 0, 0, 8, 0, 0, 0, 0, 0, 1);
+    case 11: return HX_LAUNCH_G(128, 0, 0, 0, 8, 1, 0, 0, 0, 0, 1);
     case 12: return HX_LAUNCH(128, 0, 0, 0, 8, 0, 0, 0, 0, 0, 1);
     case 13: return HX_LAUNCH(256, 1, 0, 0, 8, 0, 0, 0, 0, 0, 1);
     case 14: return HX_LAUNCH(128, 1, 0, 0, 8, 0, 0, 0, 0, 0, 1);
@@ -795,13 +804,13 @@
   return -6;
 }
 #undef HX_LAUNCH
-
-}
-
-MXR_API int mxr_conv3x3_hx32_act(const void* X, const void* Wt, const float* bias, const void* R, const void* Mk,
-                                 void* Y, const void* zpage, const ConvGeom* g, const void* tiles, int ntiles, int relu,
-                                 int accumulate, int variant, const int* act_list, const int* act_cnt,
-                                 hipStream_t stream) {
+#undef HX_LAUNCH_G
+
+}
+
+static int hx32_entry(const void* X, const void* Wt, const float* bias, const void* R, const void* Mk, void* Y,
+                      const void* zpage, const ConvGeom* g, const void* tiles, int ntiles, int relu, int accumulate,
+                      int variant, const int* act_list, const int* act_cnt, int need, hipStream_t stream) {
   if (g->cin % 32 != 0 || g->cout % 8 != 0) return -1;
   if (g->kh != 3 || g->kw != 3 || g->stride != 1 || g->pt != 1 || g->pl != 1 || g->ostride != 1) return -2;
   if (g->in_img != g->out_img || (g->M + 1) * (long long)std::max(g->cin, g->cout) >= (1LL << 31)) return -4;
@@ -811,12 +820,31 @@
   const HaloTile* t = (const HaloTile*)tiles;
   bf16_t* y = (bf16_t*)Y;
   if ((act_list == nullptr) != (act_cnt == nullptr)) return -7;
+  if (need && (act_list == nullptr || r != nullptr || accumulate)) return -7;
   if (act_list != nullptr) {
+    if (need)
+      return hx32_dispatch<2>(x, w, bias, r, mk, y, z, t, ntiles, *g, relu, accumulate, variant, stream, act_list,
+                              act_cnt);
     if (bias != nullptr || r != nullptr || relu) return -7;
     return hx32_dispatch<1>(x, w, bias, r, mk, y, z, t, ntiles, *g, relu, accumulate, variant, stream, act_list,
                             act_cnt);
   }
   return hx32_dispatch<0>(x, w, bias, r, mk, y, z, t, ntiles, *g, relu, accumulate, variant, stream, nullptr, nullptr);
+}
+
+MXR_API int mxr_conv3x3_hx32_act(const void* X, const void* Wt, const float* bias, const void* R, const void* Mk,
+                                 void* Y, const void* zpage, const ConvGeom* g, const void* tiles, int ntiles, int relu,
+                                 int accumulate, int variant, const int* act_list, const int* act_cnt,
+                                 hipStream_t stream) {
+  return hx32_entry(X, Wt, bias, R, Mk, Y, zpage, g, tiles, ntiles, relu, accumulate, variant, act_list, act_cnt, 0,
+                    stream);
+}
+
+MXR_API int mxr_conv3x3_hx32_need(const void* X, const void* Wt, const float* bias, const void* Mk, void* Y,
+                                  const void* zpage, const ConvGeom* g, const void* tiles, int ntiles, int relu,
+                                  int variant, const int* need_list, const int* need_cnt, hipStream_t stream) {
+  return hx32_entry(X, Wt, bias, nullptr, Mk, Y, zpage, g, tiles, ntiles, relu, 0, variant, need_list, need_cnt, 1,
+                    stream);
 }
 
 MXR_API int mxr_conv3x3_hx32(const void* X, const void* Wt, const float* bias, const void* R, const void* Mk,
diff --git a/csrc/kernels/row_activity.hip b/csrc/kernels/row_activity.hip
--- a/csrc/kernels/row_activity.hip
+++ b/csrc/kernels/row_activity.hip
@@ -24,6 +24,19 @@
   }
   __syncthreads();
   if (threadIdx.x == 0) mask[blockIdx.x] = (u64)bits[0] | ((u64)bits[1] << 32);
+}
+
+__global__ __launch_bounds__(256) void rows_positive_kernel(const int8_t* __restrict__ state, long long rows, int group,
+                                                            long long nw, u64* __restrict__ mask) {
+  const long long m = (long long)blockIdx.x * 256 + threadIdx.x;
+  bool pos = false;
+  if (m < rows) {
+    const int8_t* s = state + m * group;
+    for (int a = 0; a < group; ++a) pos |= s[a] == 1;
+  }
+  const u64 bal = __ballot(pos);
+  const long long word = m >> 6;
+  if ((threadIdx.x & 63) == 0 && word < nw) mask[word] = bal;
 }
 
 __device__ __forceinline__ u64 ra_bits(const u64* __restrict__ mask, long long nw, long long s, int len) {
@@ -70,11 +83,11 @@
   }
 }
 
-__device__ __forceinline__ bool ra_tile_active(const HaloTile& T, const u64* __restrict__ mask) {
+__device__ __forceinline__ bool ra_tile_active(const HaloTile& T, const u64* __restrict__ mask, int ext) {
   for (int b = 0; b < T.nbox; ++b) {
     const HaloBox& B = T.b[b];
-    const int ya = max(0, B.y0 - 1), yb = min(B.H - 1, B.y0 + B.R);
-    const int xa = max(0, B.x0 - 1), xb = min(B.W - 1, B.x0 + B.C);
+    const int ya = max(0, B.y0 - ext), yb = min(B.H - 1, B.y0 + B.R - 1 + ext);
+    const int xa = max(0, B.x0 - ext), xb = min(B.W - 1, B.x0 + B.C - 1 + ext);
     for (int yy = ya; yy <= yb; ++yy) {
       long long s = (long long)B.out_base + (long long)yy * B.W + xa;
       int len = xb - xa + 1;
@@ -91,19 +104,26 @@
   return false;
 }
 
+constexpr int RA_MAXLIST = 16;
+struct ListSel {
+  signed char which[RA_MAXLIST], ext[RA_MAXLIST];
+};
+
 __global__ __launch_bounds__(1024) void halo_active_tiles_kernel(const HaloTile* __restrict__ tiles, int ntiles,
                                                                  const u64* __restrict__ masks, long long stride,
-                                                                 int* __restrict__ lists, int* __restrict__ counts) {
+                                                                 int* __restrict__ lists, int* __restrict__ counts,
+                                                                 ListSel sel) {
   __shared__ int wcnt[16];
   __shared__ int base_s;
-  const u64* mask = masks + (long long)blockIdx.x * stride;
+  const u64* mask = masks + (long long)sel.which[blockIdx.x] * stride;
+  const int ext = sel.ext[blockIdx.x];
   int* list = lists + (long long)blockIdx.x * ntiles;
   const int lane = threadIdx.x & 63, wave = threadIdx.x >> 6;
   if (threadIdx.x == 0) base_s = 0;
   __syncthreads();
   for (int t0 = 0; t0 < ntiles; t0 += 1024) {
     const int t = t0 + threadIdx.x;
-    const bool act = t < ntiles && ra_tile_active(tiles[t], mask);
+    const bool act = t < ntiles && ra_tile_active(tiles[t], mask, ext);
     const u64 bal = __ballot(act);
     if (lane == 0) wcnt[wave] = __popcll(bal);
     __syncthreads();
@@ -135,6 +155,14 @@
   return (int)hipGetLastError();
 }
 
+MXR_API int mxr_rows_positive(const void* state, long long rows, int group, void* mask, hipStream_t stream) {
+  if (rows < 1 || group < 1) return -1;
+  const long long nw = (rows + 63) / 64;
+  if (nw > 0x7fffffffLL) return -4;
+  rows_positive_kernel<<<(unsigned)((nw + 3) / 4), 256, 0, stream>>>((const int8_t*)state, rows, group, nw, (u64*)mask);
+  return (int)hipGetLastError();
+}
+
 MXR_API int mxr_rows_dilate(const void* in, void* out, int nd, long long stride_words, const ConvGeom* g,
                             hipStream_t stream) {
   if (nd < 1 || nd > RA_MAXD || g->nlev < 1 || g->nlev > MXR_MAXLEV || g->M < 1) return -1;
@@ -146,10 +174,28 @@
   return (int)hipGetLastError();
 }
 
+MXR_API int mxr_halo_active_tiles_ext(const void* tiles, int ntiles, const void* masks, long long stride_words,
+                                      int nmask, int nlist, const int* which, const int* ext, int* lists, int* counts,
+                                      hipStream_t stream) {
+  if (ntiles < 1 || nmask < 1 || nlist < 1 || nlist > RA_MAXLIST) return -1;
+  ListSel sel = {};
+  for (int i = 0; i < nlist; ++i) {
+    if (which[i] < 0 || which[i] >= nmask || (ext[i] != 0 && ext[i] != 1)) return -1;
+    sel.which[i] = (signed char)which[i];
+    sel.ext[i] = (signed char)ext[i];
+  }
+  halo_active_tiles_kernel<<<(unsigned)nlist, 1024, 0, stream>>>((const HaloTile*)tiles, ntiles, (const u64*)masks,
+                                                                 stride_words, lists, counts, sel);
+  return (int)hipGetLastError();
+}
+
 MXR_API int mxr_halo_active_tiles(const void* tiles, int ntiles, const void* masks, long long stride_words, int nmask,
                                   int* lists, int* counts, hipStream_t stream) {
-  if (ntiles < 1 || nmask < 1) return -1;
-  halo_active_tiles_kernel<<<(unsigned)nmask, 1024, 0, stream>>>((const HaloTile*)tiles, ntiles, (const u64*)masks,
-                                                                 stride_words, lists, counts);
-  return (int)hipGetLastError();
-}
+  if (nmask < 1 || nmask > RA_MAXLIST) return -1;
+  int which[RA_MAXLIST], ext[RA_MAXLIST];
+  for (int i = 0; i < nmask; ++i) {
+    which[i] = i;
+    ext[i] = 1;
+  }
+  return mxr_halo_active_tiles_ext(tiles, ntiles, masks, stride_words, nmask, nmask, which, ext, lists, counts, stream);
+}
```

Result: faster. 584.9 images/sec, median of 6 (+3.0%).
